# IMMachinations/Task-Vector-Replication

Measured on AMD Instinct MI355X. Metric: patched-forward prompts/sec, Pythia-2.8B layer×head CIE sweep, 1–8 GPUs, higher is better.
Workload: dtype f32 (x2f16 emulation: fp32 activations as 2 fp16 planes against the checkpoint's exact fp16 weights, 2 MFMA products, fp32 accumulate); 1 GPU; pythia-2.8b CIE sweep 32x32 sites, 12 prompts/step, 4-shot, T=15, fp16-valued weights (exact-fp16 GEMMs, 2 products); parallelism=single GPU, gemm=x2f16, weights=fp16, exact16_gemms=True

## Files before the change

include/tvr.h:

```cpp
#ifndef TVR_H_
#define TVR_H_

#include <stddef.h>
#include <stdint.h>

#ifdef __cplusplus
extern "C" {
#endif

#define TVR_ABI_VERSION 11

enum tvr_status {
  TVR_OK = 0,
  TVR_ERR_INVALID = -1,
  TVR_ERR_HIP = -2,
  TVR_ERR_NOMEM = -3,
  TVR_ERR_UNSUPPORTED = -4,
  TVR_ERR_RANGE = -5,
  TVR_ERR_INTERNAL = -6
};

enum tvr_site_kind {
  TVR_SITE_NONE = 0,
  TVR_SITE_REPLACE_HEAD_ALLPOS = 1,
  TVR_SITE_ADD_ATTN_OUT_LASTPOS = 2,
  TVR_SITE_SET_RESID_PRE_POS = 3,
  TVR_SITE_REPLACE_HEADSET_ALLPOS = 4,
  TVR_SITE_REPLACE_HEADSET_LASTPOS = 5,
  TVR_SITE_SET_RESID_PRE_VEC = 6
};

typedef struct tvr_config {
  int32_t n_layers;
  int32_t d_model;
  int32_t n_heads;
  int32_t d_head;
  int32_t d_mlp;
  int32_t d_vocab;
  int32_t rotary_dim;
  int32_t n_ctx;
  float ln_eps;
  float rotary_base;
} tvr_config;

typedef struct tvr_layer_weights {
  const float* w1;
  const float* b1;
  const float* w2;
  const float* b2;
} tvr_layer_weights;

typedef struct tvr_site {
  int32_t seq;
  int32_t kind;
  int32_t layer;
  int32_t head;
  int32_t pos;
  int32_t src_seq;
  int32_t src_pos;
  int32_t vec;
  int32_t target;
} tvr_site;

typedef struct tvr_model tvr_model;
typedef struct tvr_trace tvr_trace;

const char* tvr_version(void);
int32_t tvr_abi_version(void);
const char* tvr_last_error(void);

int tvr_model_create(const tvr_config* cfg, const float* w_embed ,
                     const tvr_layer_weights* layers ,
                     const float* w_unembed_t ,
                     const float* b_unembed , tvr_model** out);
int tvr_model_destroy(tvr_model* model);

enum tvr_gemm_mode { TVR_GEMM_F32 = 0, TVR_GEMM_X3BF16 = 1, TVR_GEMM_X2F16 = 2, TVR_GEMM_BF16 = 3 };
int tvr_model_set_gemm(tvr_model* model, int32_t mode, void* stream);
int32_t tvr_model_get_gemm(const tvr_model* model);
int tvr_model_range_status(tvr_model* model, void* stream);

typedef struct {
  const uint16_t* w1;
  const uint16_t* w2;
  const float* g1;
  const float* g2;
} tvr_exact16_layer;
int tvr_model_set_exact16(tvr_model* model, const tvr_exact16_layer* layers );
int tvr_model_set_exact16_unembed(tvr_model* model, const uint16_t* wu, const float* gf);

int tvr_trace_create(tvr_model* model, int32_t max_seqs, int32_t max_tokens,
                     tvr_trace** out);
int tvr_trace_destroy(tvr_trace* trace);
int tvr_trace_flush(tvr_trace* trace, void* stream);
enum tvr_trace_hook { TVR_TRACE_RESID_PRE = 0, TVR_TRACE_Z = 1, TVR_TRACE_Q = 2, TVR_TRACE_K = 3, TVR_TRACE_V = 4 };
int tvr_trace_read(const tvr_trace* trace, int32_t what, int32_t layer, float* dst,
                   void* stream);
int32_t tvr_trace_num_tokens(const tvr_trace* trace);
int tvr_trace_capture_resid(tvr_trace* trace, const int32_t* pos, const int32_t* group,
                            int32_t n_groups, float* out, void* stream);
int tvr_trace_capture_pattern(tvr_trace* trace, const int32_t* pos, const int32_t* cls, int32_t n_classes,
                              float* out_pattern, int32_t ld, float* out_mass, void* stream);

int tvr_trace_logit_attribution(tvr_trace* trace, const int32_t* pos, const int32_t* target,
                                const int32_t* contrast, float* out_head, float* out_resid, void* stream);
int tvr_trace_logit_lens(tvr_trace* trace, const int32_t* pos, const int32_t* targets, float* out_prob,
                         int32_t* out_topk, int32_t topk, void* stream);

int tvr_forward_clean(tvr_model* model, tvr_trace* trace, const int32_t* tokens,
                      const int32_t* seq_lens, int32_t n_seq,
                      const int32_t* targets, float* out_prob,
                      int32_t* out_topk, int32_t topk, float* out_logits,
                      float* capture_zsum, void* stream);

int tvr_forward_clean_deferred(tvr_model* model, tvr_trace* trace, const int32_t* tokens,
                               const int32_t* seq_lens, int32_t n_seq,
                               const int32_t* targets, float* out_prob,
                               int32_t* out_topk, int32_t topk, void* stream);

int tvr_forward_logits(tvr_model* model, const int32_t* tokens, const float* resid_in,
                       int32_t start_layer, const int32_t* seq_lens, int32_t n_seq,
                       float* out_logits, void* stream);

int tvr_patch_sweep(tvr_model* model, tvr_trace* trace,
                    const tvr_site* sites, int32_t n_sites,
                    const float* vectors, int32_t n_vectors, float* out_prob,
                    int32_t* out_topk, int32_t topk, float* out_logits,
                    void* stream);

typedef struct tvr_head_patch { int32_t layer, head, vec; } tvr_head_patch;
int tvr_patch_sweep_sets(tvr_model* model, tvr_trace* trace,
                         const tvr_site* sites, int32_t n_sites,
                         const int32_t* set_off, const tvr_head_patch* patches,
                         const float* vectors, int32_t n_vectors, float* out_prob,
                         int32_t* out_topk, int32_t topk, float* out_logits,
                         void* stream);

int tvr_project_heads(tvr_model* model, const float* zsum ,
                      float* out , void* stream);

int tvr_gemm_f32(const float* A, int32_t lda, const float* W, int32_t ldw,
                 const float* bias, float* C, int32_t ldc, int32_t M,
                 int32_t N, int32_t K, void* stream);
int tvr_split_planes(const float* w, uint16_t* out, size_t n, void* stream);
int tvr_gemm_x3bf16(const float* A, int32_t lda, const uint16_t* W, int32_t ldw,
                    size_t wps, const float* bias, float* C, int32_t ldc,
                    int32_t M, int32_t N, int32_t K, void* stream);
int tvr_weight_planes(int32_t fmt, const float* w, float scale, uint16_t* out, size_t n,
                      void* stream);
int tvr_gemm_x2f16(const float* A, int32_t lda, const uint16_t* W, int32_t ldw,
                   size_t wps, float w_scale, const float* bias, float* C,
                   int32_t ldc, int32_t M, int32_t N, int32_t K,
                   uint32_t* range_flag, void* stream);
#define TVR_ACT_X2F16_IL 0x12
int tvr_act_rows(int32_t fmt, const float* a, int32_t lda, uint16_t* out, int32_t rows,
                 int32_t K, uint32_t* range_flag, void* stream);
int tvr_gemm_planar(int32_t fmt, const uint16_t* A, int32_t lda, const uint16_t* W,
                    int32_t ldw, size_t wps, float w_scale, const float* bias,
                    float* C, int32_t ldc, int32_t M, int32_t N, int32_t K,
                    void* stream);
int tvr_lnpre_f32(const float* x, int32_t ldx, float* y, int32_t ldy,
                  int32_t rows, int32_t d, float eps, void* stream);
typedef struct tvr_attn_seq { int32_t row0, n, p0, cache_row, q0, prefix_live; } tvr_attn_seq;
int tvr_attention(tvr_model* model, int32_t fmt, const float* qkv, const float* cache,
                  const tvr_attn_seq* seqs, int32_t n_seq, int32_t row_from, int32_t rows,
                  int32_t cache_rows, void* z, float* zf, int32_t zf_last, int32_t zf_rows,
                  const float* cos_t, const float* sin_t, void* stream);
int tvr_attention_pattern(tvr_model* model, const float* qkv, int32_t rows, const int32_t* row0,
                          const int32_t* qpos, int32_t n_seq, const int32_t* cls, int32_t n_classes,
                          float* out_pattern, int32_t ld, float* out_mass, const float* cos_t,
                          const float* sin_t, void* stream);
int tvr_head_attribution(tvr_model* model, int32_t layer, const float* z, const float* dirs, int32_t n,
                         float* out, void* stream);
int tvr_decode_rows(tvr_model* model, const float* rows, int32_t n, const int32_t* targets, float* out_prob,
                    int32_t* out_topk, int32_t topk, void* stream);
enum tvr_gemm_epi { TVR_EPI_BIAS = 0, TVR_EPI_GELU = 1, TVR_EPI_RESID = 2 };
enum tvr_gemm_form { TVR_FORM_PLAN = 0, TVR_FORM_PLAIN = 1, TVR_FORM_SPLITK = 2, TVR_FORM_TAIL = 3,
                     TVR_FORM_STREAMK = 4 };
enum tvr_gemm_slicing { TVR_SLICE_MODEL = 0, TVR_SLICE_ON = 1, TVR_SLICE_OFF = 2 };
typedef struct tvr_gemm_args {
  int32_t fmt, exact16, epi, form, form_n, form_tile, slicing, skinny;
  int32_t M, N, K, lda, ldw, ld0, n_split, ld1h;
  int32_t ps1h, raw_rows, ld_raw, mirror_rows, ldr, a2_col, a_buf_rows, out_buf_rows;
  float w_scale;
  int32_t reserved;
  uint64_t wps;
  const uint16_t* A;
  const uint16_t* a2;
  const uint16_t* W;
  const float* bias;
  float* out0;
  float* out0m;
  uint16_t* out1h;
  float* raw;
  const float* resid;
  uint32_t* range_flag;
  const int32_t* a_rows;
  const int32_t* out_rows;
} tvr_gemm_args;
int tvr_gemm_launch(tvr_model* model, const tvr_gemm_args* args, void* stream);

enum { TVR_ENTRY_FORCE_VALU = 1 };
int tvr_site_entry(tvr_model* model, const int32_t* seq_lens, int32_t n_seq, const int32_t* token_ids,
                   int32_t tokens, const float* resid, const float* z, const tvr_site* sites,
                   int32_t n_sites, const int32_t* set_off, const tvr_head_patch* patches,
                   const float* vectors, int32_t n_vectors, int32_t flags, float* out, int32_t out_rows,
                   int32_t* site_row0, int32_t* site_rows, int32_t* site_p0, void* stream);

typedef struct tvr_headset_item { int32_t row0, n_rows, first_patch, n_patches; } tvr_headset_item;
typedef struct tvr_headset_patch { int32_t head, vec; } tvr_headset_patch;
int tvr_headset_apply(tvr_model* model, int32_t fmt, const tvr_headset_item* items, int32_t n_items,
                      const tvr_headset_patch* patches, int32_t n_patches, const float* vectors,
                      int32_t n_vectors, void* a2, float* resid, int32_t rows, void* stream);

typedef struct tvr_kernel_stats {
  int64_t gemm_launches[3];
  double gemm_flops[3];
  double gemm_ms[3];
  double gemm_bytes[3];
} tvr_kernel_stats;
int tvr_profile_enable(tvr_model* model, int32_t on);
int tvr_profile_read(tvr_model* model, tvr_kernel_stats* out);

enum tvr_hbm_kind {
  TVR_HBM_ENTRY = 0,
  TVR_HBM_CAPTURE = 1,
  TVR_HBM_LNPRE = 2,
  TVR_HBM_ATTENTION = 3,
  TVR_HBM_ROW_STATS = 4,
  TVR_HBM_LIN_ENTRY = 5,
  TVR_HBM_KINDS = 6
};
typedef struct tvr_hbm_stats {
  int64_t launches[6];
  double ms[6];
  double bytes[6];
} tvr_hbm_stats;
int tvr_profile_read_hbm(tvr_model* model, tvr_hbm_stats* out);

// ... 11 lines not shown
```

task-vector-replication_amd/_lib.py:

```python
from __future__ import annotations

import ctypes
import os
from pathlib import Path

LIB_NAME = "libtvr.so"
OPS_NAME = "_tvr_ops.so"
LIB_PATH = Path(os.environ["TVR_LIB"]).resolve() if os.environ.get("TVR_LIB") else Path(__file__).resolve().parent / LIB_NAME

TVR_OK = 0
TVR_ERR_INVALID = -1
TVR_ERR_HIP = -2
TVR_ERR_NOMEM = -3
TVR_ERR_UNSUPPORTED = -4
TVR_ERR_RANGE = -5
TVR_ERR_INTERNAL = -6

TRACE_RESID_PRE = 0
TRACE_Z = 1
TRACE_Q = 2
TRACE_K = 3
TRACE_V = 4

SITE_NONE = 0
SITE_REPLACE_HEAD_ALLPOS = 1
SITE_ADD_ATTN_OUT_LASTPOS = 2
SITE_SET_RESID_PRE_POS = 3
SITE_REPLACE_HEADSET_ALLPOS = 4
SITE_REPLACE_HEADSET_LASTPOS = 5
SITE_SET_RESID_PRE_VEC = 6

c_f32p = ctypes.c_void_p
c_i32p = ctypes.c_void_p


class CLayerWeights(ctypes.Structure):
    _fields_ = [("w1", ctypes.c_void_p), ("b1", ctypes.c_void_p),
                ("w2", ctypes.c_void_p), ("b2", ctypes.c_void_p)]


class CExact16Layer(ctypes.Structure):
    _fields_ = [("w1", ctypes.c_void_p), ("w2", ctypes.c_void_p), ("g1", ctypes.c_void_p), ("g2", ctypes.c_void_p)]


class CSite(ctypes.Structure):
    _fields_ = [("seq", ctypes.c_int32), ("kind", ctypes.c_int32), ("layer", ctypes.c_int32),
                ("head", ctypes.c_int32), ("pos", ctypes.c_int32), ("src_seq", ctypes.c_int32),
                ("src_pos", ctypes.c_int32), ("vec", ctypes.c_int32), ("target", ctypes.c_int32)]


SITE_FIELDS = [f for f, _ in CSite._fields_]


class CHeadPatch(ctypes.Structure):
    _fields_ = [("layer", ctypes.c_int32), ("head", ctypes.c_int32), ("vec", ctypes.c_int32)]


class CHeadsetItem(ctypes.Structure):
    _fields_ = [("row0", ctypes.c_int32), ("n_rows", ctypes.c_int32), ("first_patch", ctypes.c_int32),
                ("n_patches", ctypes.c_int32)]


class CHeadsetPatch(ctypes.Structure):
    _fields_ = [("head", ctypes.c_int32), ("vec", ctypes.c_int32)]


ENTRY_FORCE_VALU = 1


class CAttnSeq(ctypes.Structure):
    _fields_ = [("row0", ctypes.c_int32), ("n", ctypes.c_int32), ("p0", ctypes.c_int32),
                ("cache_row", ctypes.c_int32), ("q0", ctypes.c_int32), ("prefix_live", ctypes.c_int32)]


ACT_X2F16_IL = 0x12


class CGemmArgs(ctypes.Structure):
    _fields_ = ([(n, ctypes.c_int32) for n in (
        "fmt", "exact16", "epi", "form", "form_n", "form_tile", "slicing", "skinny",
        "M", "N", "K", "lda", "ldw", "ld0", "n_split", "ld1h",
        "ps1h", "raw_rows", "ld_raw", "mirror_rows", "ldr", "a2_col", "a_buf_rows", "out_buf_rows")] +
                [("w_scale", ctypes.c_float), ("reserved", ctypes.c_int32), ("wps", ctypes.c_uint64)] +
                [(n, ctypes.c_void_p) for n in (
                    "A", "a2", "W", "bias", "out0", "out0m", "out1h", "raw", "resid", "range_flag",
                    "a_rows", "out_rows")])


EPI_BIAS, EPI_GELU, EPI_RESID = 0, 1, 2
FORM_PLAN, FORM_PLAIN, FORM_SPLITK, FORM_TAIL, FORM_STREAMK = 0, 1, 2, 3, 4
SLICE_MODEL, SLICE_ON, SLICE_OFF = 0, 1, 2


class CKernelStats(ctypes.Structure):
    _fields_ = [("gemm_launches", ctypes.c_int64 * 3), ("gemm_flops", ctypes.c_double * 3),
                ("gemm_ms", ctypes.c_double * 3), ("gemm_bytes", ctypes.c_double * 3)]


GEMM_VARIANTS = ("unembed", "qkv_mlpin", "o_mlpout")


class CHbmStats(ctypes.Structure):
    _fields_ = [("launches", ctypes.c_int64 * 6), ("ms", ctypes.c_double * 6), ("bytes", ctypes.c_double * 6)]


HBM_KINDS = ("entry", "capture", "lnpre", "attention", "row_stats", "lin_entry")

ABI_VERSION = 11

GEMM_MODES = {"f32": 0, "x3bf16": 1, "x2f16": 2, "bf16": 3}
GEMM_NAMES = {v: k for k, v in GEMM_MODES.items()}

SIGNATURES = {
    "tvr_version": (ctypes.c_char_p, []),
    "tvr_abi_version": (ctypes.c_int32, []),
    "tvr_last_error": (ctypes.c_char_p, []),
    "tvr_model_create": (ctypes.c_int, [ctypes.c_void_p, c_f32p, ctypes.POINTER(CLayerWeights),
                                        c_f32p, c_f32p, ctypes.POINTER(ctypes.c_void_p)]),
    "tvr_model_destroy": (ctypes.c_int, [ctypes.c_void_p]),
    "tvr_trace_create": (ctypes.c_int, [ctypes.c_void_p, ctypes.c_int32, ctypes.c_int32,
                                        ctypes.POINTER(ctypes.c_void_p)]),
    "tvr_trace_destroy": (ctypes.c_int, [ctypes.c_void_p]),
    "tvr_trace_flush": (ctypes.c_int, [ctypes.c_void_p, ctypes.c_void_p]),
    "tvr_trace_read": (ctypes.c_int, [ctypes.c_void_p, ctypes.c_int32, ctypes.c_int32, c_f32p,
                                      ctypes.c_void_p]),
    "tvr_trace_num_tokens": (ctypes.c_int32, [ctypes.c_void_p]),
    "tvr_trace_capture_resid": (ctypes.c_int, [ctypes.c_void_p, c_i32p, c_i32p, ctypes.c_int32, c_f32p,
                                               ctypes.c_void_p]),
    "tvr_forward_clean": (ctypes.c_int, [ctypes.c_void_p, ctypes.c_void_p, c_i32p, c_i32p, ctypes.c_int32,
                                         c_i32p, c_f32p, c_i32p, ctypes.c_int32, c_f32p, c_f32p,
                                         ctypes.c_void_p]),
    "tvr_forward_clean_deferred": (ctypes.c_int, [ctypes.c_void_p, ctypes.c_void_p, c_i32p, c_i32p, ctypes.c_int32,
                                                  c_i32p, c_f32p, c_i32p, ctypes.c_int32, ctypes.c_void_p]),
    "tvr_forward_logits": (ctypes.c_int, [ctypes.c_void_p, c_i32p, c_f32p, ctypes.c_int32, c_i32p, ctypes.c_int32,
                                          c_f32p, ctypes.c_void_p]),
    "tvr_patch_sweep": (ctypes.c_int, [ctypes.c_void_p, ctypes.c_void_p, ctypes.c_void_p, ctypes.c_int32,
                                       c_f32p, ctypes.c_int32, c_f32p, c_i32p, ctypes.c_int32, c_f32p,
                                       ctypes.c_void_p]),
    "tvr_patch_sweep_sets": (ctypes.c_int, [ctypes.c_void_p, ctypes.c_void_p, ctypes.c_void_p, ctypes.c_int32,
                                            c_i32p, ctypes.c_void_p, c_f32p, ctypes.c_int32, c_f32p, c_i32p,
                                            ctypes.c_int32, c_f32p, ctypes.c_void_p]),
    "tvr_project_heads": (ctypes.c_int, [ctypes.c_void_p, c_f32p, c_f32p, ctypes.c_void_p]),
    "tvr_gemm_f32": (ctypes.c_int, [c_f32p, ctypes.c_int32, c_f32p, ctypes.c_int32, c_f32p, c_f32p,
                                    ctypes.c_int32, ctypes.c_int32, ctypes.c_int32, ctypes.c_int32,
                                    ctypes.c_void_p]),
    "tvr_lnpre_f32": (ctypes.c_int, [c_f32p, ctypes.c_int32, c_f32p, ctypes.c_int32, ctypes.c_int32,
                                     ctypes.c_int32, ctypes.c_float, ctypes.c_void_p]),
    "tvr_workspace_bytes": (ctypes.c_size_t, [ctypes.c_void_p]),
    "tvr_model_set_gemm": (ctypes.c_int, [ctypes.c_void_p, ctypes.c_int32, ctypes.c_void_p]),
    "tvr_model_set_exact16": (ctypes.c_int, [ctypes.c_void_p, ctypes.c_void_p]),
    "tvr_model_set_exact16_unembed": (ctypes.c_int, [ctypes.c_void_p, ctypes.c_void_p, ctypes.c_void_p]),
    "tvr_model_get_gemm": (ctypes.c_int32, [ctypes.c_void_p]),
    "tvr_split_planes": (ctypes.c_int, [c_f32p, ctypes.c_void_p, ctypes.c_size_t, ctypes.c_void_p]),
    "tvr_gemm_x3bf16": (ctypes.c_int, [c_f32p, ctypes.c_int32, ctypes.c_void_p, ctypes.c_int32,
                                       ctypes.c_size_t, c_f32p, c_f32p, ctypes.c_int32, ctypes.c_int32,
                                       ctypes.c_int32, ctypes.c_int32, ctypes.c_void_p]),
    "tvr_model_range_status": (ctypes.c_int, [ctypes.c_void_p, ctypes.c_void_p]),
    "tvr_weight_planes": (ctypes.c_int, [ctypes.c_int32, c_f32p, ctypes.c_float, ctypes.c_void_p, ctypes.c_size_t,
                                         ctypes.c_void_p]),
    "tvr_gemm_x2f16": (ctypes.c_int, [c_f32p, ctypes.c_int32, ctypes.c_void_p, ctypes.c_int32,
                                      ctypes.c_size_t, ctypes.c_float, c_f32p, c_f32p, ctypes.c_int32,
                                      ctypes.c_int32, ctypes.c_int32, ctypes.c_int32, ctypes.c_void_p,
                                      ctypes.c_void_p]),
    "tvr_act_rows": (ctypes.c_int, [ctypes.c_int32, c_f32p, ctypes.c_int32, ctypes.c_void_p, ctypes.c_int32,
                                    ctypes.c_int32, ctypes.c_void_p, ctypes.c_void_p]),
    "tvr_gemm_planar": (ctypes.c_int, [ctypes.c_int32, ctypes.c_void_p, ctypes.c_int32, ctypes.c_void_p,
                                       ctypes.c_int32, ctypes.c_size_t, ctypes.c_float, c_f32p, c_f32p,
                                       ctypes.c_int32, ctypes.c_int32, ctypes.c_int32, ctypes.c_int32,
                                       ctypes.c_void_p]),
    "tvr_profile_enable": (ctypes.c_int, [ctypes.c_void_p, ctypes.c_int32]),
    "tvr_profile_read": (ctypes.c_int, [ctypes.c_void_p, ctypes.POINTER(CKernelStats)]),
    "tvr_profile_read_hbm": (ctypes.c_int, [ctypes.c_void_p, ctypes.POINTER(CHbmStats)]),
    "tvr_gemm_plan": (ctypes.c_int, [ctypes.c_int32, ctypes.c_int32, ctypes.c_int32, ctypes.c_int32, ctypes.c_int32,
                                     ctypes.c_void_p]),
    "tvr_attention": (ctypes.c_int, [ctypes.c_void_p, ctypes.c_int32, c_f32p, c_f32p, ctypes.c_void_p, ctypes.c_int32,
                                     ctypes.c_int32, ctypes.c_int32, ctypes.c_int32, ctypes.c_void_p, c_f32p,
                                     ctypes.c_int32, ctypes.c_int32, c_f32p, c_f32p, ctypes.c_void_p]),
    "tvr_attention_pattern": (ctypes.c_int, [ctypes.c_void_p, c_f32p, ctypes.c_int32, c_i32p, c_i32p, ctypes.c_int32,
                                             c_i32p, ctypes.c_int32, c_f32p, ctypes.c_int32, c_f32p, c_f32p, c_f32p,
                                             ctypes.c_void_p]),
    "tvr_trace_capture_pattern": (ctypes.c_int, [ctypes.c_void_p, c_i32p, c_i32p, ctypes.c_int32, c_f32p,
                                                 ctypes.c_int32, c_f32p, ctypes.c_void_p]),
    "tvr_gemm_launch": (ctypes.c_int, [ctypes.c_void_p, ctypes.POINTER(CGemmArgs), ctypes.c_void_p]),
    "tvr_head_attribution": (ctypes.c_int, [ctypes.c_void_p, ctypes.c_int32, c_f32p, c_f32p, ctypes.c_int32, c_f32p,
                                            ctypes.c_void_p]),
    "tvr_trace_logit_attribution": (ctypes.c_int, [ctypes.c_void_p, c_i32p, c_i32p, c_i32p, c_f32p, c_f32p,
                                                   ctypes.c_void_p]),
    "tvr_decode_rows": (ctypes.c_int, [ctypes.c_void_p, c_f32p, ctypes.c_int32, c_i32p, c_f32p, c_i32p,
                                       ctypes.c_int32, ctypes.c_void_p]),
    "tvr_trace_logit_lens": (ctypes.c_int, [ctypes.c_void_p, c_i32p, c_i32p, c_f32p, c_i32p, ctypes.c_int32,
                                            ctypes.c_void_p]),
    "tvr_site_entry": (ctypes.c_int, [ctypes.c_void_p, c_i32p, ctypes.c_int32, c_i32p, ctypes.c_int32, c_f32p, c_f32p,
                                      ctypes.c_void_p, ctypes.c_int32, c_i32p, ctypes.c_void_p, c_f32p,
                                      ctypes.c_int32, ctypes.c_int32, c_f32p, ctypes.c_int32, c_i32p, c_i32p, c_i32p,
                                      ctypes.c_void_p]),
    "tvr_headset_apply": (ctypes.c_int, [ctypes.c_void_p, ctypes.c_int32, ctypes.c_void_p, ctypes.c_int32,
                                         ctypes.c_void_p, ctypes.c_int32, c_f32p, ctypes.c_int32, ctypes.c_void_p,
                                         c_f32p, ctypes.c_int32, ctypes.c_void_p]),
}

OPS_PATH = LIB_PATH.parent / OPS_NAME
OPS = ("forward_clean", "patch_sweep", "project_heads", "forward_logits")
SET_OPS = ("patch_sweep_sets",)
RESID_OPS = ("capture_resid",)
PATTERN_OPS = ("capture_pattern",)
PATTERN_MAX_CLASSES = 64
ATTRIBUTION_OPS = ("head_attribution", "logit_attribution", "logit_lens", "decode_rows")
STATS_MAX_K = 16

_LIB = None
_OPS_LOADED = False


class EngineError(RuntimeError):
    pass


class RangeError(EngineError):
    """TVR_ERR_RANGE: an x2f16 GEMM input left the fp16 split's range (the
    results since the last check are not fp32-accurate).  The experiment
    functions retry on a path without that limit (``Model.range_fallback``)."""


def load(path: os.PathLike | str | None = None) -> ctypes.CDLL:
    global _LIB
    if _LIB is not None and path is None:
        return _LIB
    p = Path(path) if path else LIB_PATH
    if not p.exists():
        raise EngineError(f"{p} not found: the HIP engine is not built (no CPU fallback exists); "
                          "run `make -C task-vector-replication_amd/csrc`")
    lib = ctypes.CDLL(str(p))
    for name, (res, args) in SIGNATURES.items():
        fn = getattr(lib, name)
        fn.restype = res
# ... 35 lines not shown
```

task-vector-replication_amd/csrc/engine.hip:

```cpp
#include <hip/hip_runtime.h>

#include <algorithm>
#include <climits>
#include <cmath>
#include <cstdio>
#include <cstdlib>
#include <cstring>
#include <functional>
#include <map>
#include <string>
#include <tuple>
#include <vector>

#include "tvr.h"
#include "gemm_f32.hpp"
#include "attention_mfma.hpp"
#include "attention_pattern.hpp"
#include "logit_attribution.hpp"
#include "gemm_pingpong.hpp"
#include "gemm_skinny.hpp"
#include "gemm_planar.hpp"
#include "gemm_x2f16.hpp"
#include "gemm_x3bf16.hpp"
#include "kernels.hpp"
#include "lin_entry.hpp"
#include "entry_mfma.hpp"
#include "headset_patch.hpp"
#include "sweep_plan.hpp"

using namespace tvr;

namespace {

thread_local std::string g_last_error;

int fail(int code, const std::string& msg) {
  g_last_error = msg;
  return code;
}

#define TVR_HIP(expr)                                                           \
  do {                                                                          \
    hipError_t _e = (expr);                                                     \
    if (_e != hipSuccess)                                                       \
      return fail(TVR_ERR_HIP, std::string(#expr) + ": " + hipGetErrorString(_e)); \
  } while (0)

#define TVR_TRY(expr)        \
  do {                       \
    int _rc = (expr);        \
    if (_rc != TVR_OK) return _rc; \
  } while (0)

constexpr size_t kAlign = 256;
inline size_t align_up(size_t x) { return (x + kAlign - 1) & ~(kAlign - 1); }

struct Carve {
  size_t off = 0;
  template <class T>
  size_t take(size_t count) {
    const size_t at = off;
    off = align_up(off + count * sizeof(T));
    return at;
  }
};

struct Staging {
  void* buf[2] = {nullptr, nullptr};
  size_t cap[2] = {0, 0};
  hipEvent_t done[2] = {nullptr, nullptr};
  bool pending[2] = {false, false};
  int next = 0;
};

struct MatW {
  const float* f = nullptr;
  const uint16_t* x = nullptr;
  const uint16_t* h = nullptr;
  size_t wps = 0;
  float wscale = 1.0f;
  bool x16 = false;
  MatW rows(size_t elems) const {
    return {f ? f + elems : nullptr, x ? x + elems : nullptr, h ? h + elems : nullptr, wps, wscale, x16};
  }
};

using PlanKey = std::tuple<int, int, int, int, int, int>;
struct PpPlan {
  int ksplit = 1;
  int tail_base = 0;
  int tail_split = 1;
  int sk_base = -1;
  int sk_blocks = 0;
};
struct GemmForce {
  bool plan_set = false;
  PpPlan plan;
  int slicing = 0;
};
}

struct tvr_model {
  tvr_config cfg{};
  int D1 = 0;
  int K2 = 0;
  const float* w_embed = nullptr;
  std::vector<tvr_layer_weights> layers;
  const float* w_unembed_t = nullptr;
  const float* b_unembed = nullptr;
  float* rot_cos = nullptr;
  float* rot_sin = nullptr;
  const float** d_w2s = nullptr;
  int gemm_mode = TVR_GEMM_F32;
  uint16_t* planes = nullptr;
  unsigned* range_flag = nullptr;
  std::vector<MatW> w1, w2;
  std::vector<MatW> w1qk;
  MatW wu;
  char* ws = nullptr;
  size_t ws_bytes = 0;
  float* splitk_ws = nullptr;
  size_t splitk_bytes = 0;
  Staging staging;
  bool prof = false;
  struct ProfRec { hipEvent_t a, b; int epi; double flops, bytes; };
  std::vector<ProfRec> prof_recs;
  std::vector<hipEvent_t> prof_pool;
  int lin_mode = -1;
  int lin_failed_mode = -1;
  int lin_kp = 0;
  uint16_t* lin_planes = nullptr;
  float* lin_c1 = nullptr;
  std::vector<float> lin_scale;
  std::map<PlanKey, PpPlan> plans;
  bool x16 = false;
  bool act_il = true;
  std::vector<MatW> w1x, w2x;
  std::vector<const float*> g1, g2;
  MatW wux;
  const float* gf = nullptr;
};

struct tvr_trace {
  tvr_model* model = nullptr;
  int max_seqs = 0, max_tokens = 0;
  float* resid = nullptr;
  float* z = nullptr;
  float* qkv = nullptr;
  std::vector<int> seq_off, seq_len;
  std::vector<int32_t> tokens;
  int n_seq = 0, n_tokens = 0;
  bool pending = false;
  bool uncentred = false;
  std::vector<int32_t> p_targets;
  float* p_prob = nullptr;
  int32_t* p_topk = nullptr;
  int p_k = 0;
  void* p_stream = nullptr;
};

namespace {

constexpr int kFinalChunk = 1024;

int ensure_workspace(tvr_model* m, size_t bytes, hipStream_t st) {
  if (bytes <= m->ws_bytes) return TVR_OK;
  TVR_HIP(hipStreamSynchronize(st));
  if (m->ws) TVR_HIP(hipFree(m->ws));
  m->ws = nullptr;
  m->ws_bytes = 0;
  const size_t want = align_up(bytes + bytes / 8);
  if (hipMalloc(&m->ws, want) != hipSuccess) {
    m->ws = nullptr;
    (void)hipGetLastError();
    return fail(TVR_ERR_NOMEM, "workspace allocation of " + std::to_string(want) + " bytes failed");
  }
  m->ws_bytes = want;
  return TVR_OK;
}

int ensure_splitk(tvr_model* m, size_t bytes, hipStream_t st) {
  if (bytes <= m->splitk_bytes) return TVR_OK;
  TVR_HIP(hipStreamSynchronize(st));
  if (m->splitk_ws) TVR_HIP(hipFree(m->splitk_ws));
  m->splitk_ws = nullptr;
  m->splitk_bytes = 0;
  const size_t want = align_up(bytes);
  if (hipMalloc(&m->splitk_ws, want) != hipSuccess) {
    m->splitk_ws = nullptr;
    (void)hipGetLastError();
    return fail(TVR_ERR_NOMEM, "split-K workspace allocation of " + std::to_string(want) + " bytes failed");
  }
  m->splitk_bytes = want;
  return TVR_OK;
}

int upload(tvr_model* m, hipStream_t st, void* dst, const void* src, size_t bytes) {
  if (bytes == 0) return TVR_OK;
  Staging& s = m->staging;
  const int i = s.next;
  s.next ^= 1;
  if (s.pending[i]) {
    TVR_HIP(hipEventSynchronize(s.done[i]));
    s.pending[i] = false;
  }
  if (s.cap[i] < bytes) {
    if (s.buf[i]) TVR_HIP(hipHostFree(s.buf[i]));
    s.buf[i] = nullptr;
    const size_t want = align_up(std::max(bytes, (size_t)1 << 20));
    TVR_HIP(hipHostMalloc(&s.buf[i], want, hipHostMallocDefault));
    s.cap[i] = want;
  }
  if (!s.done[i]) TVR_HIP(hipEventCreateWithFlags(&s.done[i], hipEventDisableTiming));
  std::memcpy(s.buf[i], src, bytes);
  TVR_HIP(hipMemcpyAsync(dst, s.buf[i], bytes, hipMemcpyHostToDevice, st));
  TVR_HIP(hipEventRecord(s.done[i], st));
  s.pending[i] = true;
  return TVR_OK;
}

struct UploadBatch {
  std::vector<char> host;
  struct Item { size_t host_off; size_t dev_off; size_t bytes; };
  std::vector<Item> items;
  template <class T>
  void add(size_t dev_off, const std::vector<T>& v) {
    items.push_back({host.size(), dev_off, v.size() * sizeof(T)});
    const char* p = reinterpret_cast<const char*>(v.data());
    host.insert(host.end(), p, p + v.size() * sizeof(T));
  }
};

int flush_uploads(tvr_model* m, hipStream_t st, char* base, const UploadBatch& ub) {
  if (ub.items.empty()) return TVR_OK;
  const size_t first = ub.items.front().dev_off;
  std::vector<char> span;
  size_t end = first;
  for (const auto& it : ub.items) end = std::max(end, it.dev_off + it.bytes);
  span.assign(end - first, 0);
  for (const auto& it : ub.items)
    std::memcpy(span.data() + (it.dev_off - first), ub.host.data() + it.host_off, it.bytes);
  return upload(m, st, base + first, span.data(), span.size());
}

hipEvent_t prof_event(tvr_model* m) {
  hipEvent_t e = nullptr;
  if (!m->prof_pool.empty()) {
    e = m->prof_pool.back();
    m->prof_pool.pop_back();
  } else if (hipEventCreate(&e) != hipSuccess) {
    e = nullptr;
  }
  return e;
}

struct ProfSpan {
  tvr_model* m;
  hipStream_t st;
  hipEvent_t a = nullptr, b = nullptr;
  ProfSpan(tvr_model* m_, hipStream_t s) : m(m_), st(s) {
    if (m && m->prof) {
      a = prof_event(m);
      b = prof_event(m);
      if (a) (void)hipEventRecord(a, st);
    }
  }
  void done(int kind, double bytes) {
    if (!a || !b) return;
    (void)hipEventRecord(b, st);
    m->prof_recs.push_back({a, b, 3 + kind, 0.0, bytes});
    a = b = nullptr;
  }
  ~ProfSpan() {
    if (a) m->prof_pool.push_back(a);
    if (b) m->prof_pool.push_back(b);
  }
};

bool env_flag(const char* name) {
  const char* e = getenv(name);
  return !(e && std::string(e) == "0");
}
bool prefix_share_enabled() { return env_flag("TVR_PREFIX_SHARE"); }
bool lin_entry_enabled() { return env_flag("TVR_LIN_ENTRY"); }

int act_fmt(const tvr_model* m) {
  return m->gemm_mode == TVR_GEMM_X2F16 ? ACT_X2F16 : m->gemm_mode == TVR_GEMM_BF16 ? ACT_BF16 : ACT_F32;
}

bool use_x16(const tvr_model* m) { return m->x16 && m->gemm_mode == TVR_GEMM_X2F16; }

bool act_layout_interleaved() {
  const char* e = getenv("TVR_ACT_LAYOUT");
  return !(e && std::string(e) == "planar");
}
int acts_fmt(const tvr_model* m) { return use_x16(m) && m->act_il ? (int)ACT_X2F16I : act_fmt(m); }

int env_int(const char* name, int dflt) {
  const char* e = getenv(name);
  return e && *e ? atoi(e) : dflt;
}
int pp_group_m(int N) {
  static const int small = env_int("TVR_PP_GM_SMALL", 2), large = env_int("TVR_PP_GM_LARGE", 4);
  return (N + 255) / 256 <= 16 ? small : large;
}

void launch_pp(PpKernel kp, const uint16_t* Ah, int lda, const MatW& W, int ldw, int M, int N, int K,
               const GemmEpi& ep0, float acc_scale, int tile_base, int count, hipStream_t st) {
  GemmEpi ep = ep0;
  ep.tile_base = tile_base;
  ep.tile_count = count;
  ep.group_m = pp_group_m(N);
  const dim3 g(count > 0 ? count : gemm_pingpong_grid(M, N));
  hipLaunchKernelGGL(kp, g, dim3(PP_THREADS), 0, st, Ah, 2 * lda, (size_t)lda, W.h, ldw, W.wps, acc_scale, M, N, K, ep);
}

struct PpLaunch {
  PpKernel whole = nullptr;
  PpKernel partial = nullptr;
  PpReduceKernel reduce = nullptr;
  PpSkReduceKernel sk_reduce = nullptr;
  bool skm = false;
  int base = 0, n = 0;
};

int launch_pp_partial(const PpLaunch& pl, const uint16_t* Ah, int lda, int a_fmt, const MatW& W, int ldw, int M, int N,
                      int K, const GemmEpi& ep0, float acc_scale, int count, tvr_model* m, hipStream_t st) {
  const int n = pl.n;
  const size_t ws_tiles = pl.skm ? (size_t)2 * n : (size_t)n * count;
  const int rc = ensure_splitk(m, ws_tiles * PP_TILE_ELEMS * sizeof(float), st);
  if (rc != TVR_OK) return rc;
  GemmEpi ep = ep0;
  ep.group_m = pp_group_m(N);
  GemmEpi pe{};
  pe.group_m = ep.group_m;
  pe.out0 = m->splitk_ws;
  pe.a_rows = ep.a_rows;
  if (pl.skm) pe.sk_blocks = n; else pe.k_split = n;
  pe.tile_base = pl.base;
  pe.tile_count = count;
  pe.a2 = ep.a2;
  pe.a2_col = ep.a2_col;
  const dim3 g(pl.skm ? n : count * n);
  const dim3 rg((unsigned)std::min<long>(4096, ((long)count * (PP_TILE_ELEMS / 4) + 255) / 256));
  hipLaunchKernelGGL(pl.partial, g, dim3(PP_THREADS), 0, st, Ah, 2 * lda, (size_t)lda, W.h, ldw, W.wps, acc_scale, M,
                     N, K, pe);
  const float* part = (const float*)m->splitk_ws;
  if (pl.skm)
    hipLaunchKernelGGL(pl.sk_reduce, rg, dim3(256), 0, st, part, n, K / pp_ktile(a_fmt), pl.base, count, M, N, ep);
  else
    hipLaunchKernelGGL(pl.reduce, rg, dim3(256), 0, st, part, n, pl.base, count, M, N, ep);
  return TVR_OK;
}

int sk_mode() {
  const char* e = getenv("TVR_STREAM_K");
  return !e ? 0 : std::string(e) == "1" ? 1 : std::string(e) == "O" ? 2 : 0;
}
bool sk_enabled(int epi = EPI_BIAS) {
  const int md = sk_mode();
  return md == 1 || (md == 2 && epi == EPI_RESID);
}

struct PlanCost {
  double kt_us, pro_us, epi_us, part_us;
};

double plan_sim(int M, int N, int nkt, int t0, int cnt, int S, const PlanCost& pc) {
  const int nbm = (M + 255) / 256, nbn = (N + 255) / 256, gm = pp_group_m(N);
  const int nb = cnt * S, P = 256;
  std::vector<double> cu(P, 0.0);
  auto remap = [](int bid, int nwg) {
    const int xcd = bid & 7, q = nwg >> 3, r = nwg & 7;
    return (xcd < r ? xcd * (q + 1) : r * (q + 1) + (xcd - r) * q) + (bid >> 3);
  };
  double end = 0.0;
  for (int b = 0; b < nb; ++b) {
// ... 29 lines not shown
  PpPlan p;
  const int tiles = gemm_pingpong_grid(M, N), nkt = K / pp_ktile(a_fmt);
  const double kt_scale = wx ? (sliced ? 0.85 : 0.72) : 1.0;
  const double kt_us = (a_fmt == ACT_X2F16 ? 1.9 : 1.3) * (sliced ? 1.13 : 1.0) * kt_scale, seg_us = 15.0,
               epi_us = 10.0;
  auto sk_us = [&](int cnt) {
    const int G = (int)std::min<long long>(256, (long long)cnt * nkt);
    return std::ceil((double)cnt * nkt / G) * kt_us + 2.0 * seg_us + (cnt + 2.0 * G) * 0.0655 + 5.0;
  };
  const double round_plain_us = nkt * kt_us + epi_us;
  if (sk_enabled(epi) && (long long)tiles * nkt >= 4LL * 256) {
    const int rounds = (tiles + 255) / 256;
    const int tb = tiles - 256 * (rounds - 1);
    if (tb < 256 && sk_us(tb) + 5.0 < round_plain_us) {
      p.sk_base = tiles - tb;
      p.sk_blocks = (int)std::min<long long>(256, (long long)tb * nkt);
      return p;
    }
  }
  if (tiles <= 1024) {
    const PlanCost pc{kt_us, 3.0, epi == EPI_SPLIT_GELU_ACT ? 15.0 : 10.0, 7.0};
    double best = plan_sim(M, N, nkt, 0, tiles, 1, pc);
    for (int S = 2; S <= 16 && nkt / S >= 8 && tiles * S <= 4096; ++S) {
      const double c = plan_sim(M, N, nkt, 0, tiles, S, pc) + plan_reduce_us(M, N, 0, tiles, S);
      if (c < best * 0.97) {
        best = c;
        p.ksplit = S;
      }
    }
    if (tiles > 256) {
      const int base = 256 * ((tiles - 1) / 256), cnt = tiles - base;
      const double head = plan_sim(M, N, nkt, 0, base, 1, pc);
      for (int S = 2; S <= 16 && nkt / S >= 8; ++S) {
        const double c = head + plan_sim(M, N, nkt, base, cnt, S, pc) + plan_reduce_us(M, N, base, cnt, S);
        if (c < best * 0.97) {
          best = c;
          p.ksplit = 1;
          p.tail_base = base;
          p.tail_split = S;
        }
      }
    }
    return p;
  }
  const int rounds = (tiles + 255) / 256;
  const int tb = tiles - 256 * (rounds - 1);
  if (tb > 224) return p;
  int best = 1;
  double br = 1.0;
  for (int s = 2; s <= 16 && nkt / s >= 8; ++s) {
    const double r = std::ceil(tb * (double)s / 256.0) / s;
    if (r < br - 1e-9) {
      br = r;
      best = s;
    }
  }
  if (best < 2) return p;
  const double round_us = nkt * 2.5 * kt_scale;
  const double saved_us = (1.0 - br) * round_us;
  const double cost_us = (best + 1.0) * tb * (double)PP_TILE_ELEMS * 8.0 / 5.0e6;
  if (saved_us > 1.5 * cost_us + 10.0) {
    p.tail_base = 256 * (rounds - 1);
    p.tail_split = best;
  }
  return p;
}

PpPlan plan_pp_cached(tvr_model* m, int M, int N, int K, int a_fmt, int epi, bool wx = false) {
  const PlanKey key{M, N, K, a_fmt + (wx ? 16 : 0), epi == EPI_SPLIT_GELU_ACT ? 1 : epi == EPI_RESID ? 2 : 0, sk_mode()};
  auto it = m->plans.find(key);
  if (it != m->plans.end()) return it->second;
  const PpPlan p = plan_pp(M, N, K, a_fmt, epi, a_fmt == ACT_X2F16 && pp_sliced_rule(K, m->K2), wx);
  if (m->plans.size() > 4096) m->plans.clear();
  m->plans.emplace(key, p);
  return p;
}

int resolve_pp(const PpForm& f, const PpPlan& plan, PpLaunch& pl) {
  auto missing = [](const char* what, const PpForm& g) {
    return fail(TVR_ERR_INTERNAL, std::string("gemm: no ") + what + " is instantiated for the form epi " +
                                      std::to_string(g.epi) + ", fmt " + std::to_string(g.fmt) + ", vec " +
                                      std::to_string(g.vec) + ", stream-K " + std::to_string(g.skm) + ", sliced " +
                                      std::to_string(g.sl) + ", one weight plane " + std::to_string(g.wx) +
                                      ", interleaved A " + std::to_string(g.ail));
  };
  pl.skm = plan.sk_base >= 0;
  const bool whole_split = !pl.skm && plan.ksplit > 1, tail_split = !pl.skm && !whole_split && plan.tail_base > 0;
  pl.base = pl.skm ? plan.sk_base : tail_split ? plan.tail_base : 0;
  pl.n = pl.skm ? plan.sk_blocks : whole_split ? plan.ksplit : tail_split ? plan.tail_split : 0;
  if (pl.n == 0 || pl.base > 0) {
    PpForm whole = f;
    whole.vec = f.vec || pl.n > 0;
    pl.whole = pp_kernel(whole);
    if (!pl.whole) return missing("gemm_pingpong_kernel", whole);
  }
  if (pl.n > 0) {
    PpForm part = f;
    part.epi = EPI_BIAS;
    part.vec = true;
    part.skm = pl.skm;
    pl.partial = pp_kernel(part);
    if (!pl.partial) return missing("partial-tile gemm_pingpong_kernel", part);
    const int out_fmt = pp_reduce_fmt(f.fmt, f.ail);
    if (pl.skm)
      pl.sk_reduce = pp_reduce_kernel<true>(f.epi, out_fmt);
    else
      pl.reduce = pp_reduce_kernel<false>(f.epi, out_fmt);
    if (!pl.sk_reduce && !pl.reduce) return missing("reduce kernel", part);
  }
  return TVR_OK;
}

int launch_gemm(int epi, const void* A, int lda, int a_fmt, const MatW& W, int ldw, int M, int N,
                int K, const GemmEpi& ep, hipStream_t st, tvr_model* m = nullptr,
                unsigned* range_flag = nullptr, const GemmForce* force = nullptr) {
  if (M <= 0 || N <= 0) return TVR_OK;
  const bool ail = a_fmt == ACT_X2F16I;
  if (ail) {
    a_fmt = ACT_X2F16;
    if (!W.x16 && (epi != EPI_BIAS || m || ep.skinny))
      return fail(TVR_ERR_INVALID, "gemm: the interleaved activation layout belongs to the one-plane exact-fp16 GEMMs");
  }
  const bool planar = a_fmt != ACT_F32;
  if (planar && !W.h) return fail(TVR_ERR_INVALID, "gemm: planar activations need the planar weight planes");
  if (epi == EPI_SPLIT_GELU_ACT && !planar)
    return fail(TVR_ERR_INVALID, "gemm: the activation-format GELU epilogue belongs to the planar paths");
  if (epi == EPI_SPLIT_GELU && planar)
    return fail(TVR_ERR_INVALID, "gemm: planar paths write GELU columns in their activation format");
  if (epi == EPI_STATS && (!planar || N % 4 != 0 || !ep.stats))
    return fail(TVR_ERR_INVALID, "gemm: the fused statistics epilogue needs a planar format, N % 4 == 0 and a "
                                 "statistics buffer");
  if (a_fmt == ACT_F16 && epi != EPI_BIAS)
    return fail(TVR_ERR_INVALID, "gemm: the fp16 operand format has the plain (bias) epilogue only");
  if (W.x16 && a_fmt != ACT_X2F16)
    return fail(TVR_ERR_INVALID, "gemm: one-plane exact fp16 weights take x2f16 activations");
  if (ep.a2 && (a_fmt == ACT_F32 || ep.a2_col % 256 != 0))
    return fail(TVR_ERR_INVALID, "gemm: a second A operand needs a planar format and a 256-column boundary");
  if (K % GEMM_BK != 0 || lda % 4 != 0 || ldw % 4 != 0 || ((W.x || W.h) && ldw % 8 != 0) ||
      ((a_fmt == ACT_BF16 || a_fmt == ACT_F16) && K % 64 != 0))
    return fail(TVR_ERR_UNSUPPORTED, "gemm: K, lda, ldw must be multiples of 32/4/4 (8 for planes, K of 64 for "
                                     "bf16; K=" + std::to_string(K) + ")");
  const bool wx = a_fmt == ACT_X2F16 && W.x16;
  bool vec = false, sl = false, skinny = false;
  PpLaunch pl;
  if (planar) {
    vec = planar_epilogue_vec(epi, ep, N);
    static const int wx_slice = env_int("TVR_WX_SLICE", 1);
    sl = force && force->slicing ? a_fmt == ACT_X2F16 && force->slicing == 1
                                 : a_fmt == ACT_X2F16 && pp_sliced_rule(K, m ? m->K2 : 0) &&
                                       (!wx || wx_slice == 1 || (wx_slice == 2 && epi == EPI_RESID));
    skinny = ep.skinny && epi == EPI_BIAS && M <= SK_USE_M && !ep.out_rows && ep.k_split <= 1 && vec &&
             a_fmt != ACT_F16 && !wx && !ep.a2 && !ail;
    if (!skinny) {
      PpPlan plan;
      if (force && force->plan_set)
        plan = force->plan;
      else if (m && vec && epi != EPI_STATS)
        plan = plan_pp_cached(m, M, N, K, a_fmt, epi, wx);
      TVR_TRY(resolve_pp(PpForm{epi, a_fmt, vec || epi == EPI_STATS, false, sl, wx, ail}, plan, pl));
    }
  }
  hipEvent_t ev0 = nullptr, ev1 = nullptr;
  if (m && m->prof) {
    ev0 = prof_event(m);
    ev1 = prof_event(m);
    if (ev0) TVR_HIP(hipEventRecord(ev0, st));
  }
  const float acc_scale = a_fmt == ACT_BF16 ? 1.0f : a_fmt == ACT_F16 ? 1.0f / W.wscale : 1.0f / (W.wscale * X2_ASCALE);
  if (planar) {
    const uint16_t* Ah = static_cast<const uint16_t*>(A);
    if (skinny) {
      const dim3 g(gemm_skinny_grid(N));
#define TVR_SK(F, MT)                                                                                  \
  hipLaunchKernelGGL((gemm_skinny_kernel<F, MT>), g, dim3(SK_THREADS), 0, st, Ah, 2 * lda, (size_t)lda, W.h, \
                     ldw, W.wps, acc_scale, M, N, K, ep)
#define TVR_SK_F(F)                     \
  switch ((M + 15) / 16) {              \
    case 1: TVR_SK(F, 1); break;        \
    case 2: TVR_SK(F, 2); break;        \
    case 3: TVR_SK(F, 3); break;        \
    default: TVR_SK(F, 4); break;       \
  }
      if (a_fmt == ACT_X2F16) { TVR_SK_F(ACT_X2F16); } else { TVR_SK_F(ACT_BF16); }
#undef TVR_SK_F
#undef TVR_SK
    } else {
      if (pl.n == 0 || pl.base > 0) launch_pp(pl.whole, Ah, lda, W, ldw, M, N, K, ep, acc_scale, 0, pl.base, st);
      if (pl.n > 0)
        TVR_TRY(launch_pp_partial(pl, Ah, lda, a_fmt, W, ldw, M, N, K, ep, acc_scale,
                                  gemm_pingpong_grid(M, N) - pl.base, m, st));
    }
  } else {
    const float* Af = static_cast<const float*>(A);
    unsigned* flag = m ? m->range_flag : range_flag;
    const bool f32_sliced = !W.h && !W.x && pp_sliced_rule(K, m ? m->K2 : 0);
    const bool large = gemm_use_large(M, N) && !f32_sliced;
#define TVR_GEMM_LAUNCH(E, TL)                                                                                    \
  do {                                                                                                            \
    if (f32_sliced)                                                                                               \
      hipLaunchKernelGGL((gemm_f32_nt_kernel<E, TileSmall, F32_SLICE_KT>), dim3(gemm_grid<TileSmall>(M, N)),      \
                         dim3(TileSmall::THREADS), 0, st, Af, lda, W.f, ldw, M, N, K, ep);                        \
    else                                                                                                          \
      hipLaunchKernelGGL((gemm_f32_nt_kernel<E, TL>), dim3(gemm_grid<TL>(M, N)), dim3(TL::THREADS), 0,             \
                         st, Af, lda, W.f, ldw, M, N, K, ep);                                                     \
  } while (0)
#define TVR_X3_LAUNCH(E, TL)                                                                      \
  hipLaunchKernelGGL((gemm_x3bf16_nt_kernel<E, TL>), dim3(gemm_x3_grid<TL>(M, N)), dim3(TL::THREADS), \
                     0, st, Af, lda, W.x, ldw, W.wps, M, N, K, ep)
#define TVR_X2_LAUNCH(E, TL)                                                                         \
  hipLaunchKernelGGL((gemm_x2f16_nt_kernel<E, TL>), dim3(gemm_x2_grid<TL>(M, N)), dim3(TL::THREADS), 0, \
                     st, Af, lda, W.h, ldw, W.wps, acc_scale, flag, M, N, K, ep)
#define TVR_GEMM_PICK(E)                                                          \
  if (W.h) {                                                                      \
    if (large) TVR_X2_LAUNCH(E, X2Large); else TVR_X2_LAUNCH(E, X2Small);         \
  } else if (W.x) {                                                               \
    if (large) TVR_X3_LAUNCH(E, X3Large); else TVR_X3_LAUNCH(E, X3Small);         \
  } else {                                                                        \
    if (large) TVR_GEMM_LAUNCH(E, TileLarge); else TVR_GEMM_LAUNCH(E, TileSmall); \
  }
    switch (epi) {
      case EPI_BIAS: TVR_GEMM_PICK(EPI_BIAS); break;
      case EPI_SPLIT_GELU: TVR_GEMM_PICK(EPI_SPLIT_GELU); break;
      default: TVR_GEMM_PICK(EPI_RESID); break;
    }
#undef TVR_GEMM_PICK
#undef TVR_X2_LAUNCH
#undef TVR_X3_LAUNCH
#undef TVR_GEMM_LAUNCH
  }
  TVR_HIP(hipGetLastError());
  if (ev0 && ev1) {
    TVR_HIP(hipEventRecord(ev1, st));
    const double wbytes = W.x ? 6.0 : (a_fmt == ACT_BF16 || a_fmt == ACT_F16 ? 2.0 : 4.0);
    const double abytes = a_fmt == ACT_BF16 || a_fmt == ACT_F16 ? 2.0 : 4.0;
    const double cbytes = epi == EPI_STATS ? 4.0 * M * (double)ep.stats_tiles * (2 + 2 * ep.stats_k)
                                           : 4.0 * M * (double)N;
    const int kind = epi == EPI_SPLIT_GELU_ACT ? (int)EPI_SPLIT_GELU : epi == EPI_STATS ? (int)EPI_BIAS : epi;
    m->prof_recs.push_back({ev0, ev1, kind, 2.0 * M * N * (double)K,
                            abytes * M * (double)K + cbytes + wbytes * N * (double)K});
  }
  return TVR_OK;
}

int lin_qk_cols(const tvr_config& c) { return (2 * c.d_model) % 256 == 0 ? 2 * c.d_model : 0; }

int ensure_lin(tvr_model* m, hipStream_t st) {
  const int fmt = act_fmt(m);
  if (fmt == ACT_F32) return fail(TVR_ERR_INVALID, "lin entry: needs a planar GEMM mode");
  if (m->lin_planes && m->lin_mode == m->gemm_mode) return TVR_OK;
  if (m->lin_failed_mode == m->gemm_mode)
    return fail(TVR_ERR_NOMEM, "lin entry: the W1 W_O planes do not fit (earlier attempt)");
  const tvr_config& c = m->cfg;
  const int L = c.n_layers, d = c.d_model, H = c.n_heads, dh = c.d_head, N = m->D1;
  if (L < 3) return fail(TVR_ERR_INVALID, "lin entry: needs >= 3 layers");
  TVR_HIP(hipStreamSynchronize(st));
  if (m->lin_planes) TVR_HIP(hipFree(m->lin_planes));
  if (m->lin_c1) TVR_HIP(hipFree(m->lin_c1));
  m->lin_planes = nullptr;
  m->lin_c1 = nullptr;
  const int KP = (dh + 31) / 32 * 32, npl = fmt == ACT_X2F16 ? 2 : 1;
  const size_t per = (size_t)H * N * KP;
  float *wt = nullptr, *sc = nullptr;
  unsigned* d_max = nullptr;
  auto cleanup = [&]() {
    if (wt) (void)hipFree(wt);
    if (sc) (void)hipFree(sc);
    if (d_max) (void)hipFree(d_max);
  };
  const size_t splitk_had = m->splitk_bytes;
  for (int attempt = 0;; ++attempt) {
    bool ok = hipMalloc(&m->lin_planes, (size_t)(L - 2) * npl * per * sizeof(uint16_t)) == hipSuccess &&
              hipMalloc(&m->lin_c1, (size_t)L * N * sizeof(float)) == hipSuccess &&
              hipMalloc(&wt, (size_t)d * d * sizeof(float)) == hipSuccess &&
              hipMalloc(&sc, (size_t)N * d * sizeof(float)) == hipSuccess &&
              hipMalloc(&d_max, sizeof(unsigned)) == hipSuccess;
    if (ok && attempt > 0 && splitk_had > 0) {
      (void)hipGetLastError();
      ok = hipMalloc(&m->splitk_ws, splitk_had) == hipSuccess;
      if (ok) {
        m->splitk_bytes = splitk_had;
      } else {
        m->splitk_ws = nullptr;
      }
    }
    if (ok) break;
    (void)hipGetLastError();
    cleanup();
    wt = sc = nullptr;
    d_max = nullptr;
    if (m->lin_planes) (void)hipFree(m->lin_planes);
    if (m->lin_c1) (void)hipFree(m->lin_c1);
    m->lin_planes = nullptr;
    m->lin_c1 = nullptr;
    if (attempt == 0 && m->splitk_ws) {
      (void)hipFree(m->splitk_ws);
      m->splitk_ws = nullptr;
      m->splitk_bytes = 0;
      continue;
    }
    m->lin_failed_mode = m->gemm_mode;
    return fail(TVR_ERR_NOMEM, "lin entry: the W1 W_O planes do not fit");
  }
  m->lin_scale.assign(L, 1.0f);
  int rc = TVR_OK;
  for (int l = 1; l <= L - 2 && rc == TVR_OK; ++l) {
    hipLaunchKernelGGL(transpose_kernel, dim3((d + 31) / 32, (d + 31) / 32), dim3(32, 8), 0, st,
                       m->layers[l - 1].w2, m->K2, wt, d);
    GemmEpi e{};
    e.out0 = sc;
    e.ld0 = d;
    rc = launch_gemm(EPI_BIAS, m->layers[l].w1, d, ACT_F32, MatW{wt}, d, N, d, d, e, st);
    if (rc != TVR_OK) break;
    float scale = 1.0f;
    {
      unsigned hm = 0;
      hipError_t e2 = hipMemsetAsync(d_max, 0, sizeof(unsigned), st);
      if (e2 == hipSuccess) {
        const size_t n_abs = fmt == ACT_X2F16 ? (size_t)N * d : (size_t)2 * d * d;
        hipLaunchKernelGGL(absmax_kernel, dim3(1024), dim3(256), 0, st, sc, n_abs, d_max);
        e2 = hipGetLastError();
      }
      if (e2 == hipSuccess) e2 = hipMemcpyAsync(&hm, d_max, sizeof(unsigned), hipMemcpyDeviceToHost, st);
      if (e2 == hipSuccess) e2 = hipStreamSynchronize(st);
// ... 189 lines not shown
  const float inv_scale = 1.0f / std::sqrt((float)dh);
  const dim3 grid((unsigned)(n_seq * c.n_heads), (unsigned)n_layers), block(64);
#define TVR_PATTERN(DHV)                                                                                          \
  hipLaunchKernelGGL((attention_pattern_kernel<DHV>), grid, block, lds, st, qkv, layer_stride, 3 * d, d_seqs,      \
                     c.n_heads, d_cls, n_classes, out_pattern, ld, out_mass, rot_cos, rot_sin, d, inv_scale)
  if (dh == 16) { TVR_PATTERN(16); } else if (dh == 64) { TVR_PATTERN(64); }
  else if (dh == 80) { TVR_PATTERN(80); } else { TVR_PATTERN(128); }
#undef TVR_PATTERN
  TVR_HIP(hipGetLastError());
  return TVR_OK;
}

int check_pattern_args(const char* fn, const int32_t* cls, int n_cls, int32_t n_classes, const float* out_pattern,
                       const float* out_mass) {
  auto bad = [&](const std::string& what) { return fail(TVR_ERR_INVALID, std::string(fn) + ": " + what); };
  if (!out_pattern && !out_mass) return bad("out_pattern and out_mass are both null");
  if (out_mass && !cls) return bad("out_mass needs cls");
  if (cls) {
    if (n_classes <= 0 || n_classes > PATTERN_MAX_CLASSES)
      return bad("n_classes must be in [1, " + std::to_string(PATTERN_MAX_CLASSES) + "]");
    for (int r = 0; r < n_cls; ++r)
      if (cls[r] < -1 || cls[r] >= n_classes)
        return bad("class of row " + std::to_string(r) + " outside [-1, n_classes)");
  }
  return TVR_OK;
}

int launch_head_attribution(tvr_model* m, const char* fn, const float* dirs, int n, const float* z, size_t z_lstride,
                            const int32_t* d_zrows, int layer0, int n_layers, float* out, hipStream_t st) {
  const tvr_config& c = m->cfg;
  const int d = c.d_model, dh = c.d_head, H = c.n_heads;
  const int chunks = (n + ATTR_CHUNK - 1) / ATTR_CHUNK;
  if (!(dh == 16 || dh == 64 || dh == 80 || dh == 128) || d % 16 != 0)
    return fail(TVR_ERR_UNSUPPORTED, std::string(fn) + ": the attribution kernel covers d_head 16 / 64 / 80 / 128");
  if (H > 65535 || n_layers > 65535)
    return fail(TVR_ERR_UNSUPPORTED, std::string(fn) + ": too many heads or layers for one launch");
  ProfSpan ps(m, st);
  const dim3 grid((unsigned)chunks, (unsigned)H, (unsigned)n_layers), block(64 * ATTR_WAVES);
#define TVR_ATTR(NT)                                                                                              \
  hipLaunchKernelGGL((head_attribution_kernel<NT>), grid, block, 0, st, dirs, n, z, z_lstride, d_zrows, m->d_w2s, \
                     layer0, m->K2, out, n_layers, H, d)
  if (dh == 16) { TVR_ATTR(1); } else if (dh == 64) { TVR_ATTR(4); }
  else if (dh == 80) { TVR_ATTR(5); } else { TVR_ATTR(8); }
#undef TVR_ATTR
  TVR_HIP(hipGetLastError());
  ps.done(TVR_HBM_CAPTURE, 4.0 * n_layers * ((double)chunks * d * d + 2.0 * n * d + (double)n * H));
  return TVR_OK;
}

GemmEpi epi_qkv_mlpin(tvr_model* m, const float* b1, float* qkv, const Acts& a) {
  const bool planar = a.fmt != ACT_F32;
  const int d = m->cfg.d_model;
  GemmEpi e{};
  e.bias = b1;
  e.out0 = qkv;
  e.ld0 = 3 * d;
  e.n_split = 3 * d;
  e.out0m = a.qkv_mirror;
  e.mirror_rows = a.mirror_rows;
  if (planar) {
    e.out1h = reinterpret_cast<uint16_t*>(a.a2) + act_col_rt(a.fmt, d);
    e.ld1h = 2 * m->K2;
    e.ps1h = m->K2;
    e.range_flag = m->range_flag;
  } else {
    e.out1 = a.a2 + d;
    e.ld1 = m->K2;
  }
  return e;
}

double attention_bytes(int d, int q_rows, int kv_rows, int fmt, int zf_rows) {
  return ((double)q_rows * d + 2.0 * kv_rows * d) * 4.0 + (double)q_rows * d * (fmt == ACT_BF16 ? 2.0 : 4.0) +
         (double)zf_rows * d * 4.0;
}

int launch_w1(tvr_model* m, int l, const void* xn, int M, int c0, int N, const GemmEpi& ep, hipStream_t st,
              const void* xn2 = nullptr) {
  const int d = m->cfg.d_model;
  const int fmt = xn2 ? acts_fmt(m) : act_fmt(m);
  const int epi = fmt != ACT_F32 ? EPI_SPLIT_GELU_ACT : EPI_SPLIT_GELU;
  if (xn2) {
    if (!use_x16(m) || !act_is_x2(fmt)) return fail(TVR_ERR_INTERNAL, "launch_w1: gamma-scaled rows off the x16 path");
    const MatW W = m->w1x[l].rows((size_t)c0 * d);
    const int qkv_end = 3 * d - c0;
    if (qkv_end <= 0)
      return launch_gemm(epi, xn2, d, fmt, W, d, M, N, d, ep, st, m);
    if (qkv_end >= N)
      return launch_gemm(epi, xn, d, fmt, W, d, M, N, d, ep, st, m);
    if (qkv_end % 256 == 0) {
      GemmEpi e = ep;
      e.a2 = static_cast<const uint16_t*>(xn2);
      e.a2_col = qkv_end;
      return launch_gemm(epi, xn, d, fmt, W, d, M, N, d, e, st, m);
    }
    GemmEpi e1 = ep;
    e1.n_split = std::min(ep.n_split, qkv_end);
    TVR_TRY(launch_gemm(epi, xn, d, fmt, W, d, M, qkv_end, d, e1, st, m));
    GemmEpi e2 = ep;
    e2.bias = ep.bias ? ep.bias + qkv_end : nullptr;
    e2.out0 = ep.out0 ? ep.out0 + qkv_end : nullptr;
    if (ep.out0m) e2.out0m = ep.out0m + qkv_end;
    e2.n_split = ep.n_split - qkv_end;
    if (e2.n_split < 0) return fail(TVR_ERR_INTERNAL, "launch_w1: MLP-in columns below the GELU split");
    return launch_gemm(epi, xn2, d, fmt, W.rows((size_t)qkv_end * d), d, M, N - qkv_end, d, e2, st, m);
  }
  const int nqk = fmt == ACT_BF16 && !m->w1qk.empty() ? std::min(std::max(2 * d - c0, 0), N) : 0;
  if (nqk > 0) {
    GemmEpi e{};
    e.bias = ep.bias;
    e.out0 = ep.out0;
    e.ld0 = ep.ld0;
    e.a_rows = ep.a_rows;
    e.out_rows = ep.out_rows;
    e.out0m = ep.out0m;
    e.mirror_rows = ep.mirror_rows;
    TVR_TRY(launch_gemm(EPI_BIAS, static_cast<const uint16_t*>(xn) + d, d, ACT_F16,
                        m->w1qk[l].rows((size_t)c0 * d), d, M, nqk, d, e, st, m));
    if (nqk == N) return TVR_OK;
  }
  GemmEpi e = ep;
  if (nqk > 0) {
    e.bias = ep.bias ? ep.bias + nqk : nullptr;
    e.out0 = ep.out0 + nqk;
    if (ep.out0m) e.out0m = ep.out0m + nqk;
    e.n_split = ep.n_split - nqk;
  }
  return launch_gemm(epi, xn, d, fmt, m->w1[l].rows((size_t)(c0 + nqk) * d), d, M, N - nqk, d, e, st, m);
}

int apply_headset(tvr_model* m, const Acts& a, hipStream_t st) {
  if (a.hs_n <= 0) return TVR_OK;
  const tvr_config& c = m->cfg;
  const int d = c.d_model;
  const bool planar = a.fmt != ACT_F32;
  const size_t row_bytes = (size_t)m->K2 * 4;
  const int slice_bytes = c.d_head * (planar ? 2 : 4);
  const int n_planes = act_is_x2(a.fmt) ? 2 : 1;
  const int il = a.fmt == ACT_X2F16I;
  const size_t plane_bytes = (size_t)m->K2 * 2;
  const dim3 g(a.hs_n, (a.hs_max_rows + HEADSET_ROWS - 1) / HEADSET_ROWS);
  const bool v4 = ((uintptr_t)a.hs_vectors & 15) == 0 && d % 4 == 0;
  ProfSpan ps(m, st);
  if (v4)
    hipLaunchKernelGGL(headset_patch_kernel<true>, g, dim3(HEADSET_THREADS), 0, st, a.hs_items, a.hs_patches,
                       a.hs_vectors, (char*)a.a2, row_bytes, slice_bytes, n_planes, plane_bytes, a.resid, d, il);
  else
    hipLaunchKernelGGL(headset_patch_kernel<false>, g, dim3(HEADSET_THREADS), 0, st, a.hs_items, a.hs_patches,
                       a.hs_vectors, (char*)a.a2, row_bytes, slice_bytes, n_planes, plane_bytes, a.resid, d, il);
  TVR_HIP(hipGetLastError());
  ps.done(TVR_HBM_ENTRY, a.hs_bytes);
  return TVR_OK;
}

int run_block(tvr_model* m, int l, int R, const SeqDesc* d_seqs, int n_seqs, int maxT,
              Acts& a, float* qkv_out, const float* cache_qkv, float* zf, hipStream_t st, bool zf_last = false,
              int zf_rows = INT_MAX, int row_from = INT_MAX) {
  const tvr_config& c = m->cfg;
  const int d = c.d_model;
  const tvr_layer_weights& w = m->layers[l];
  TVR_TRY(launch_lnpre(a.resid, d, nullptr, a.xn, d, R, d, c.ln_eps, a.fmt, st, m, nullptr, a.resid_mirror,
                       a.mirror_rows, a.xn2 ? m->g1[l] : nullptr, a.xn2 ? m->g2[l] : nullptr, a.xn2));
  const GemmEpi e1 = epi_qkv_mlpin(m, w.b1, qkv_out, a);
  TVR_TRY(launch_w1(m, l, a.xn, R, 0, m->D1, e1, st, a.xn2));
  ProfSpan ps(m, st);
  TVR_TRY(launch_attention(m, qkv_out, cache_qkv, d_seqs, n_seqs, maxT, a.a2, a.fmt, zf, st, zf_last, zf_rows,
                           row_from));
  ps.done(TVR_HBM_ATTENTION, attention_bytes(d, R, R, a.fmt, zf ? (zf_last ? n_seqs : std::min(R, zf_rows)) : 0));
  return TVR_OK;
}

int run_block_last_rows(tvr_model* m, int l, int R, const SeqDesc* d_seqs, int n_seqs, int maxT, Acts& a,
                        const float* cache_qkv, const int32_t* d_last, int n_last, bool write_out,
                        float* zf, hipStream_t st, bool zf_last = false, int zf_rows = INT_MAX, int row_from = 0) {
  const tvr_config& c = m->cfg;
  const int d = c.d_model;
  const tvr_layer_weights& w = m->layers[l];
  TVR_TRY(launch_lnpre(a.resid, d, nullptr, a.xn, d, R, d, c.ln_eps, a.fmt, st, m, nullptr, a.resid_mirror,
                       a.mirror_rows, a.xn2 ? m->g1[l] : nullptr, a.xn2 ? m->g2[l] : nullptr, a.xn2));
  GemmEpi kv{};
  kv.bias = w.b1 + d;
  kv.out0 = a.qkv + d;
  kv.ld0 = 3 * d;
  kv.n_split = 2 * d;
  TVR_TRY(launch_w1(m, l, a.xn, R, d, 2 * d, kv, st, a.xn2));
  GemmEpi e1 = epi_qkv_mlpin(m, w.b1, a.qkv, a);
  e1.a_rows = d_last;
  e1.out_rows = d_last;
// ... 97 lines not shown
  return TVR_OK;
}

int check_config(const tvr_config& c) {
  if (c.n_layers <= 0 || c.d_model <= 0 || c.n_heads <= 0 || c.d_head <= 0 || c.d_mlp <= 0 ||
      c.d_vocab <= 0 || c.n_ctx <= 0)
    return fail(TVR_ERR_INVALID, "config: all sizes must be positive");
  if (c.n_heads * c.d_head != c.d_model)
    return fail(TVR_ERR_INVALID, "config: n_heads * d_head must equal d_model");
  if (c.rotary_dim < 0 || c.rotary_dim > c.d_head || (c.rotary_dim & 1))
    return fail(TVR_ERR_INVALID, "config: rotary_dim must be even and <= d_head");
  if (c.d_model % GEMM_BK != 0 || (c.d_model + c.d_mlp) % GEMM_BK != 0)
    return fail(TVR_ERR_UNSUPPORTED, "config: d_model and d_model + d_mlp must be multiples of 32");
  if (!(c.d_head == 16 || c.d_head == 64 || c.d_head == 80 || c.d_head == 128) || c.rotary_dim * 4 != c.d_head)
    return fail(TVR_ERR_UNSUPPORTED, "config: the attention kernel covers the Pythia heads: d_head 16 / 64 / 80 / "
                                     "128 with rotary_dim = d_head / 4");
  return TVR_OK;
}

}

namespace {
int flush_pending(tvr_trace* t, void* stream);
}

extern "C" {

const char* tvr_version(void) {
  return "tvr-mi355x 0.5.0 (gfx950, fp32 MFMA | fp32-accurate 3-plane bf16 / 2-plane fp16 split MFMA | bf16 MFMA)";
}
int32_t tvr_abi_version(void) { return TVR_ABI_VERSION; }
const char* tvr_last_error(void) { return g_last_error.c_str(); }

int tvr_model_create(const tvr_config* cfg, const float* w_embed, const tvr_layer_weights* layers,
                     const float* w_unembed_t, const float* b_unembed, tvr_model** out) {
  if (!cfg || !w_embed || !layers || !w_unembed_t || !out)
    return fail(TVR_ERR_INVALID, "tvr_model_create: null argument");
  TVR_TRY(check_config(*cfg));
  for (int l = 0; l < cfg->n_layers; ++l)
    if (!layers[l].w1 || !layers[l].b1 || !layers[l].w2 || !layers[l].b2)
      return fail(TVR_ERR_INVALID, "tvr_model_create: null weight in layer " + std::to_string(l));
  auto* m = new tvr_model();
  m->cfg = *cfg;
  m->D1 = 3 * cfg->d_model + cfg->d_mlp;
  m->K2 = cfg->d_model + cfg->d_mlp;
  m->w_embed = w_embed;
  m->layers.assign(layers, layers + cfg->n_layers);
  m->w_unembed_t = w_unembed_t;
  m->b_unembed = b_unembed;
  for (int l = 0; l < cfg->n_layers; ++l) {
    m->w1.push_back(MatW{layers[l].w1});
    m->w2.push_back(MatW{layers[l].w2});
  }
  m->wu = MatW{w_unembed_t};
  const int rd = std::max(cfg->rotary_dim, 2), n_ctx = cfg->n_ctx;
  std::vector<float> hc((size_t)n_ctx * rd), hs((size_t)n_ctx * rd);
  const int half = rd / 2;
  for (int p = 0; p < n_ctx; ++p)
    for (int i = 0; i < rd; ++i) {
      const float dim = (float)(i % half);
      const float freq = std::pow(cfg->rotary_base, dim / (float)half);
      const float ang = (float)p / freq;
      hc[(size_t)p * rd + i] = std::cos(ang);
      hs[(size_t)p * rd + i] = std::sin(ang);
    }
  std::vector<const float*> w2s(cfg->n_layers);
  for (int l = 0; l < cfg->n_layers; ++l) w2s[l] = layers[l].w2;
  hipError_t e = hipMalloc(&m->rot_cos, hc.size() * sizeof(float));
  if (e == hipSuccess) e = hipMalloc(&m->rot_sin, hs.size() * sizeof(float));
  if (e == hipSuccess) e = hipMalloc(&m->d_w2s, w2s.size() * sizeof(float*));
  if (e == hipSuccess) e = hipMalloc(&m->range_flag, sizeof(unsigned));
  if (e == hipSuccess) e = hipMemset(m->range_flag, 0, sizeof(unsigned));
  if (e == hipSuccess) e = hipMemcpy(m->rot_cos, hc.data(), hc.size() * sizeof(float), hipMemcpyHostToDevice);
  if (e == hipSuccess) e = hipMemcpy(m->rot_sin, hs.data(), hs.size() * sizeof(float), hipMemcpyHostToDevice);
  if (e == hipSuccess) e = hipMemcpy(m->d_w2s, w2s.data(), w2s.size() * sizeof(float*), hipMemcpyHostToDevice);
  if (e != hipSuccess) {
    tvr_model_destroy(m);
    return fail(TVR_ERR_HIP, std::string("tvr_model_create: ") + hipGetErrorString(e));
  }
  *out = m;
  return TVR_OK;
}

int tvr_model_destroy(tvr_model* m) {
  if (!m) return TVR_OK;
  (void)hipDeviceSynchronize();
  if (m->rot_cos) (void)hipFree(m->rot_cos);
  if (m->rot_sin) (void)hipFree(m->rot_sin);
  if (m->d_w2s) (void)hipFree(m->d_w2s);
  if (m->planes) (void)hipFree(m->planes);
  if (m->lin_planes) (void)hipFree(m->lin_planes);
  if (m->lin_c1) (void)hipFree(m->lin_c1);
  if (m->range_flag) (void)hipFree(m->range_flag);
  if (m->ws) (void)hipFree(m->ws);
  if (m->splitk_ws) (void)hipFree(m->splitk_ws);
  for (auto& r : m->prof_recs) {
    (void)hipEventDestroy(r.a);
    (void)hipEventDestroy(r.b);
  }
  for (auto e : m->prof_pool) (void)hipEventDestroy(e);
  for (int i = 0; i < 2; ++i) {
    if (m->staging.buf[i]) (void)hipHostFree(m->staging.buf[i]);
    if (m->staging.done[i]) (void)hipEventDestroy(m->staging.done[i]);
  }
  delete m;
  return TVR_OK;
}

size_t tvr_workspace_bytes(const tvr_model* m) { return m ? m->ws_bytes : 0; }

int32_t tvr_model_get_gemm(const tvr_model* m) { return m ? m->gemm_mode : -1; }

static int replan_x2f16(tvr_model* m) {
  if (m->gemm_mode != TVR_GEMM_X2F16) return TVR_OK;
  TVR_HIP(hipDeviceSynchronize());
  TVR_TRY(tvr_model_set_gemm(m, TVR_GEMM_F32, nullptr));
  return tvr_model_set_gemm(m, TVR_GEMM_X2F16, nullptr);
}

int tvr_model_set_exact16_unembed(tvr_model* m, const uint16_t* wu, const float* gf) {
  if (!m) return fail(TVR_ERR_INVALID, "tvr_model_set_exact16_unembed: null model");
  if (!wu != !gf) return fail(TVR_ERR_INVALID, "tvr_model_set_exact16_unembed: give both arrays or neither");
  m->wux = wu ? MatW{nullptr, nullptr, wu, 0, 1.0f, true} : MatW{};
  m->gf = gf;
  return TVR_OK;
}

int tvr_model_set_exact16(tvr_model* m, const tvr_exact16_layer* layers) {
  if (!m) return fail(TVR_ERR_INVALID, "tvr_model_set_exact16: null model");
  const tvr_config& c = m->cfg;
  if (!layers) {
    const bool was = m->x16;
    m->x16 = false;
    m->w1x.clear();
    m->w2x.clear();
    m->g1.clear();
    m->g2.clear();
    return was ? replan_x2f16(m) : TVR_OK;
  }
  for (int l = 0; l < c.n_layers; ++l)
    if (!layers[l].w1 || !layers[l].w2 || !layers[l].g1 || !layers[l].g2)
      return fail(TVR_ERR_INVALID, "tvr_model_set_exact16: null array in layer " + std::to_string(l));
  if (c.d_model % 32 != 0 || m->K2 % 32 != 0)
    return fail(TVR_ERR_UNSUPPORTED, "tvr_model_set_exact16: d_model and d_model + d_mlp must be multiples of 32");
  m->w1x.clear();
  m->w2x.clear();
  m->g1.clear();
  m->g2.clear();
  for (int l = 0; l < c.n_layers; ++l) {
    m->w1x.push_back(MatW{nullptr, nullptr, layers[l].w1, 0, 1.0f, true});
    m->w2x.push_back(MatW{nullptr, nullptr, layers[l].w2, 0, 1.0f, true});
    m->g1.push_back(layers[l].g1);
    m->g2.push_back(layers[l].g2);
  }
  m->x16 = true;
  return replan_x2f16(m);
}

int tvr_model_set_gemm(tvr_model* m, int32_t mode, void* stream) {
  if (!m) return fail(TVR_ERR_INVALID, "tvr_model_set_gemm: null model");
  if (mode != TVR_GEMM_F32 && mode != TVR_GEMM_X3BF16 && mode != TVR_GEMM_X2F16 && mode != TVR_GEMM_BF16)
    return fail(TVR_ERR_INVALID, "tvr_model_set_gemm: unknown mode " + std::to_string(mode));
  if (mode == m->gemm_mode) return TVR_OK;
  if (mode == TVR_GEMM_BF16 && (m->cfg.d_model % 64 != 0 || m->K2 % 64 != 0))
    return fail(TVR_ERR_UNSUPPORTED, "tvr_model_set_gemm: bf16 needs d_model and d_model + d_mlp multiples of 64");
  const hipStream_t st = (hipStream_t)stream;
  TVR_HIP(hipStreamSynchronize(st));
  for (auto& w : m->w1) w = MatW{w.f};
  for (auto& w : m->w2) w = MatW{w.f};
  m->w1qk.clear();
  m->wu = MatW{m->wu.f};
  if (m->planes) TVR_HIP(hipFree(m->planes));
  m->planes = nullptr;
  if (m->lin_planes) TVR_HIP(hipFree(m->lin_planes));
  if (m->lin_c1) TVR_HIP(hipFree(m->lin_c1));
  m->lin_planes = nullptr;
  m->lin_c1 = nullptr;
  m->lin_mode = -1;
  m->lin_failed_mode = -1;
  m->gemm_mode = TVR_GEMM_F32;
  if (mode == TVR_GEMM_F32) return TVR_OK;

  const tvr_config& c = m->cfg;
  const int L = c.n_layers;
  const size_t n1 = (size_t)m->D1 * c.d_model, n2 = (size_t)c.d_model * m->K2;
  const size_t nu = (size_t)c.d_vocab * c.d_model;
  const int np = mode == TVR_GEMM_X3BF16 ? 3 : mode == TVR_GEMM_X2F16 ? 2 : 1;
  const size_t nqk = (size_t)2 * c.d_model * c.d_model;
  const bool bf16_qk16 = env_int("TVR_DEBUG_BF16_QK", 1) != 0;
  const bool bf16_trunc = env_int("TVR_DEBUG_BF16_TRUNC", 0) != 0;
  const size_t total = np * ((mode == TVR_GEMM_X2F16 && m->x16 ? 0 : n1 + n2) * L + nu) +
                       (mode == TVR_GEMM_BF16 && bf16_qk16 ? nqk * L : 0);
  if (hipMalloc(&m->planes, total * sizeof(uint16_t)) != hipSuccess) {
    m->planes = nullptr;
    (void)hipGetLastError();
    return fail(TVR_ERR_NOMEM, "tvr_model_set_gemm: weight planes (" + std::to_string(total * 2) +
                                   " bytes) do not fit");
  }
  const bool skip_x16 = mode == TVR_GEMM_X2F16 && m->x16;
  std::vector<MatW*> mats;
  std::vector<size_t> sizes;
  for (int l = 0; l < L && !skip_x16; ++l) {
    mats.push_back(&m->w1[l]);
    sizes.push_back(n1);
    mats.push_back(&m->w2[l]);
    sizes.push_back(n2);
  }
  mats.push_back(&m->wu); sizes.push_back(nu);
  if (mode == TVR_GEMM_BF16 && bf16_qk16) {
    for (int l = 0; l < L; ++l) {
      mats.push_back(nullptr);
      sizes.push_back(nqk);
    }
  }
  std::vector<float> scale(mats.size(), 1.0f);
  size_t planned = 0;
  for (size_t i = 0; i < mats.size(); ++i) planned += (mats[i] ? (size_t)np : 1) * sizes[i];
  auto drop_planes = [&]() {
    (void)hipFree(m->planes);
    m->planes = nullptr;
    for (auto& w : m->w1) w = MatW{w.f};
    for (auto& w : m->w2) w = MatW{w.f};
    m->w1qk.clear();
    m->wu = MatW{m->wu.f};
  };
  if (planned != total) {
    drop_planes();
    return fail(TVR_ERR_INTERNAL, "tvr_model_set_gemm: planes planned " + std::to_string(planned) +
                                      " != allocated " + std::to_string(total));
  }
  if (mode == TVR_GEMM_X2F16 || mode == TVR_GEMM_BF16) {
    unsigned* d_max = nullptr;
    TVR_HIP(hipMalloc(&d_max, mats.size() * sizeof(unsigned)));
    std::vector<unsigned> h_max(mats.size(), 0);
    hipError_t e = hipMemsetAsync(d_max, 0, mats.size() * sizeof(unsigned), st);
    for (size_t i = 0; i < mats.size() && e == hipSuccess; ++i) {
      const float* src = mats[i] ? mats[i]->f : m->w1[i - (mats.size() - L)].f;
      if (mode == TVR_GEMM_BF16 && mats[i]) continue;
      hipLaunchKernelGGL(absmax_kernel, dim3(1024), dim3(256), 0, st, src, sizes[i], d_max + i);
      e = hipGetLastError();
    }
    if (e == hipSuccess) e = hipMemcpyAsync(h_max.data(), d_max, mats.size() * sizeof(unsigned),
                                            hipMemcpyDeviceToHost, st);
    if (e == hipSuccess) e = hipStreamSynchronize(st);
    (void)hipFree(d_max);
    if (e != hipSuccess) return fail(TVR_ERR_HIP, std::string("tvr_model_set_gemm: ") + hipGetErrorString(e));
    for (size_t i = 0; i < mats.size(); ++i) {
      float v;
      std::memcpy(&v, &h_max[i], sizeof(v));
      scale[i] = x2_weight_scale(v);
    }
  }
  uint16_t* p = m->planes;
  for (size_t i = 0; i < mats.size(); ++i) {
    const size_t n = sizes[i];
    if (!mats[i]) {
      const int l = (int)(i - (mats.size() - L));
      const float* f = m->w1[l].f;
      hipLaunchKernelGGL(f16_plane_kernel, dim3(2048), dim3(256), 0, st, f, scale[i], p, n);
      TVR_HIP(hipGetLastError());
      m->w1qk.push_back(MatW{f, nullptr, p, n, scale[i]});
      p += n;
      continue;
    }
    MatW& w = *mats[i];
    if (mode == TVR_GEMM_X3BF16) {
      hipLaunchKernelGGL(split_planes_kernel, dim3(2048), dim3(256), 0, st, w.f, p, n);
      w = MatW{w.f, p, nullptr, n, 1.0f};
    } else if (mode == TVR_GEMM_BF16) {
      hipLaunchKernelGGL(bf16_plane_kernel, dim3(2048), dim3(256), 0, st, w.f, p, n, (int)bf16_trunc);
      w = MatW{w.f, nullptr, p, n, 1.0f};
    } else {
      hipLaunchKernelGGL(split_planes_f16_kernel, dim3(2048), dim3(256), 0, st, w.f, scale[i], p, n);
      w = MatW{w.f, nullptr, p, n, scale[i]};
    }
    TVR_HIP(hipGetLastError());
    p += np * n;
  }
  if ((size_t)(p - m->planes) != total) {
    (void)hipStreamSynchronize(st);
    const size_t written = (size_t)(p - m->planes);
    drop_planes();
    return fail(TVR_ERR_INTERNAL, "tvr_model_set_gemm: planes written " + std::to_string(written) +
                                      " != allocated " + std::to_string(total));
  }
  TVR_HIP(hipMemsetAsync(m->range_flag, 0, sizeof(unsigned), st));
  TVR_HIP(hipStreamSynchronize(st));
  m->gemm_mode = mode;
  m->act_il = act_layout_interleaved();
  return TVR_OK;
}

int tvr_model_range_status(tvr_model* m, void* stream) {
  if (!m) return fail(TVR_ERR_INVALID, "tvr_model_range_status: null model");
  const hipStream_t st = (hipStream_t)stream;
  unsigned h = 0;
  TVR_HIP(hipMemcpyAsync(&h, m->range_flag, sizeof(unsigned), hipMemcpyDeviceToHost, st));
  TVR_HIP(hipStreamSynchronize(st));
  if (h == 0) return TVR_OK;
  TVR_HIP(hipMemsetAsync(m->range_flag, 0, sizeof(unsigned), st));
  TVR_HIP(hipStreamSynchronize(st));
  return fail(TVR_ERR_RANGE, "a GEMM input reached |a| >= " + std::to_string((int)(X2_FP16_OVERFLOW / X2_ASCALE)) +
                                 ", outside the fp16-split (X2F16) range; results since the last check are not "
                                 "fp32-accurate: use gemm mode x3bf16 or f32");
}

int tvr_profile_enable(tvr_model* m, int32_t on) {
  if (!m) return fail(TVR_ERR_INVALID, "tvr_profile_enable: null model");
  TVR_HIP(hipDeviceSynchronize());
  for (auto& r : m->prof_recs) {
    m->prof_pool.push_back(r.a);
    m->prof_pool.push_back(r.b);
  }
  m->prof_recs.clear();
  m->prof = on != 0;
  return TVR_OK;
}

int tvr_profile_read(tvr_model* m, tvr_kernel_stats* out) {
  if (!m || !out) return fail(TVR_ERR_INVALID, "tvr_profile_read: null argument");
  tvr_kernel_stats s{};
  for (auto& r : m->prof_recs) {
    if (r.epi >= 3) continue;
    TVR_HIP(hipEventSynchronize(r.b));
    float ms = 0.f;
    TVR_HIP(hipEventElapsedTime(&ms, r.a, r.b));
    s.gemm_launches[r.epi] += 1;
    s.gemm_flops[r.epi] += r.flops;
    s.gemm_bytes[r.epi] += r.bytes;
    s.gemm_ms[r.epi] += ms;
  }
  *out = s;
  return TVR_OK;
}

int tvr_profile_read_hbm(tvr_model* m, tvr_hbm_stats* out) {
  if (!m || !out) return fail(TVR_ERR_INVALID, "tvr_profile_read_hbm: null argument");
  tvr_hbm_stats s{};
  for (auto& r : m->prof_recs) {
    if (r.epi < 3) continue;
    TVR_HIP(hipEventSynchronize(r.b));
    float ms = 0.f;
    TVR_HIP(hipEventElapsedTime(&ms, r.a, r.b));
    const int k = r.epi - 3;
    s.launches[k] += 1;
    s.ms[k] += ms;
    s.bytes[k] += r.bytes;
  }
  *out = s;
  return TVR_OK;
}

int tvr_trace_create(tvr_model* m, int32_t max_seqs, int32_t max_tokens, tvr_trace** out) {
  if (!m || !out || max_seqs <= 0 || max_tokens <= 0)
    return fail(TVR_ERR_INVALID, "tvr_trace_create: bad argument");
  const tvr_config& c = m->cfg;
  auto* t = new tvr_trace();
  t->model = m;
  t->max_seqs = max_seqs;
  t->max_tokens = max_tokens;
  const size_t per = (size_t)max_tokens * c.d_model * sizeof(float);
  hipError_t e = hipMalloc(&t->resid, per * (c.n_layers + 1));
  if (e == hipSuccess) e = hipMalloc(&t->z, per * c.n_layers);
  if (e == hipSuccess) e = hipMalloc(&t->qkv, per * 3 * c.n_layers);
  if (e != hipSuccess) {
    (void)hipGetLastError();
    tvr_trace_destroy(t);
    return fail(TVR_ERR_NOMEM, "tvr_trace_create: device allocation failed");
  }
  *out = t;
  return TVR_OK;
}

// ... 577 lines not shown
                       bool force_valu = false) {
  tvr_model* m = cx.m;
  const SweepPlan& p = cx.p;
  const tvr_config& c = m->cfg;
  const int d = c.d_model, k0 = l > 0 ? p.cnt_le[l - 1] : 0, k1 = p.cnt_le[l];
  if (k1 <= k0) return TVR_OK;
  const float* snap = cx.fused ? cx.a.resid : resid_base + (size_t)l * tstride;
  const float* zsnap = l > 0 ? z_base + (size_t)(l - 1) * tstride : nullptr;
  const float* w2 = l > 0 ? m->layers[l - 1].w2 : nullptr;
  const dim3 eg(k1 - k0, (d + ENTRY_THREADS - 1) / ENTRY_THREADS);
  ProfSpan ps(m, cx.st);
  const bool mf = !force_valu && p.eg_cnt[l] > 0 &&
                  (c.d_head == 16 || c.d_head == 64 || c.d_head == 80 || c.d_head == 128);
  if (mf) {
    const dim3 gg(p.eg_cnt[l], (d + ENTRY_COLS - 1) / ENTRY_COLS);
#define TVR_ENTRY_MF(DH)                                                                                     \
  hipLaunchKernelGGL(entry_replace_mfma_kernel<DH>, gg, dim3(ENTRY_THREADS), 0, cx.st, cx.ents, cx.egidx,     \
                     cx.egroups + p.eg_beg[l], snap, zsnap, w2, m->K2, cx.vectors, cx.a.resid, d)
    switch (c.d_head) {
      case 16: TVR_ENTRY_MF(16); break;
      case 64: TVR_ENTRY_MF(64); break;
      case 80: TVR_ENTRY_MF(80); break;
      default: TVR_ENTRY_MF(128); break;
    }
#undef TVR_ENTRY_MF
    TVR_HIP(hipGetLastError());
  }
  if (p.ent_other[l] || !mf) {
    const size_t zbytes = mf ? 0 : (size_t)std::min(p.maxT, ENTRY_LDS_POS) * c.d_head * sizeof(float);
    if (zbytes > 64 * 1024)
      TVR_HIP(hipFuncSetAttribute((const void*)entry_kernel, hipFuncAttributeMaxDynamicSharedMemorySize,
                                  (int)zbytes));
    hipLaunchKernelGGL(entry_kernel, eg, dim3(ENTRY_THREADS), zbytes, cx.st, cx.ents + k0, snap, zsnap, w2, m->K2,
                       cx.vectors, cx.a.resid, d, c.d_head, mf ? 1 : 0);
    TVR_HIP(hipGetLastError());
  }
  ps.done(TVR_HBM_ENTRY, p.entry_bytes[l]);
  return TVR_OK;
}

static int sweep_block_lin(const SweepCtx& cx, int l, int Rl, const float* cache, float* zf) {
  tvr_model* m = cx.m;
  const SweepPlan& p = cx.p;
  Acts& a = cx.a;
  hipStream_t st = cx.st;
  const tvr_config& c = m->cfg;
  const tvr_layer_weights& w = m->layers[l];
  const int d = c.d_model, fmt = act_fmt(m), Rc = p.Rc, Rp = Rc + p.rows_le[l - 1], D1 = m->D1, nv = p.lin_nv[l];
  const int32_t* vids = cx.lin_vids + p.lin_vid_off[l];
  TVR_TRY(launch_lnpre(a.resid, d, nullptr, a.xn, d, Rl, d, c.ln_eps, a.fmt, st, m, cx.lnstats, a.resid_mirror,
                       a.mirror_rows, a.xn2 ? m->g1[l] : nullptr, a.xn2 ? m->g2[l] : nullptr, a.xn2));
  GemmEpi e1 = epi_qkv_mlpin(m, w.b1, a.qkv, a);
  e1.raw = cx.raw_h;
  e1.raw_rows = Rc;
  e1.ld_raw = c.d_mlp;
  TVR_TRY(launch_w1(m, l, a.xn, Rp, 0, D1, e1, st, a.xn2));
  ProfSpan ps(m, st);
  const bool prof = m->prof;
  m->prof = false;
  GemmEpi eg{};
  eg.out0 = cx.g;
  eg.ld0 = D1;
  eg.a_rows = vids;
  eg.skinny = 1;
  int rc = TVR_OK;
  const int nqk = fmt == ACT_BF16 && !m->w1qk.empty() ? 2 * d : 0;
  if (use_x16(m)) {
    uint16_t* vg1 = cx.vg;
    uint16_t* vg2 = vg1 + (size_t)2 * nv * d;
    hipLaunchKernelGGL(lin_gamma_rows_kernel, dim3((nv + 3) / 4), dim3(256), 0, st, cx.vectors, d, vids, m->g1[l],
                       m->g2[l], vg1, vg2, nv, m->range_flag);
    rc = hipGetLastError() == hipSuccess ? TVR_OK : fail(TVR_ERR_HIP, "lin_gamma_rows_kernel launch");
    GemmEpi ex = eg;
    ex.a_rows = nullptr;
    const int q = 3 * d;
    if (rc == TVR_OK && q % 256 == 0) {
      ex.a2 = vg2;
      ex.a2_col = q;
      rc = launch_gemm(EPI_BIAS, vg1, d, fmt, m->w1x[l], d, nv, D1, d, ex, st, m);
    } else if (rc == TVR_OK) {
      rc = launch_gemm(EPI_BIAS, vg1, d, fmt, m->w1x[l], d, nv, q, d, ex, st, m);
      GemmEpi e2 = ex;
      e2.out0 = ex.out0 + q;
      if (rc == TVR_OK)
        rc = launch_gemm(EPI_BIAS, vg2, d, fmt, m->w1x[l].rows((size_t)q * d), d, nv, D1 - q, d, e2, st, m);
    }
  } else if (nqk > 0) {
    rc = launch_gemm(EPI_BIAS, cx.vact + d, d, ACT_F16, m->w1qk[l], d, nv, nqk, d, eg, st, m);
    GemmEpi e2 = eg;
    e2.out0 = eg.out0 + nqk;
    if (rc == TVR_OK)
      rc = launch_gemm(EPI_BIAS, cx.vact, d, fmt, m->w1[l].rows((size_t)nqk * d), d, nv, D1 - nqk, d, e2, st, m);
  } else {
    rc = launch_gemm(EPI_BIAS, cx.vact, d, fmt, m->w1[l], d, nv, D1, d, eg, st, m);
  }
  m->prof = prof;
  TVR_TRY(rc);
  const int npl = fmt == ACT_X2F16 ? 2 : 1, KP = m->lin_kp, nmb = p.lin_nmb[l];
  const size_t per = (size_t)c.n_heads * D1 * KP;
  const uint16_t* wp = m->lin_planes + (size_t)(l - 1) * npl * per;
  const int n_ct = (D1 + 255) / 256, ct_qk = fmt == ACT_BF16 ? lin_qk_cols(c) / 256 : 0;
  float acc_scale = fmt == ACT_X2F16 ? 1.0f / (m->lin_scale[l] * X2_ASCALE) : 1.0f;
  dim3 g;
  int ct_base = 0;
#define TVR_LIN(F, NK, ...)                                                                                          \
  hipLaunchKernelGGL((lin_entry_kernel<F, NK __VA_OPT__(,) __VA_ARGS__>), g, dim3(LIN_THREADS), 0, st,                \
                     cx.lin_mbs + p.lin_mb_off[l], nmb, cx.lin_rows, wp, per, acc_scale,                              \
                     cx.trace->z + (size_t)(l - 1) * cx.trace->max_tokens * d, d, c.d_head, cx.lnstats, a.qkv,        \
                     cx.raw_h, c.d_mlp, cx.g, m->lin_c1 + (size_t)l * D1, w.b1, D1,                                   \
                     reinterpret_cast<uint16_t*>(a.a2) + act_col_rt(a.fmt, d), 2 * m->K2, m->K2, m->range_flag, ct_base)
#define TVR_LIN_K(F, ...)                                                 \
  if (KP == 32) TVR_LIN(F, 1 __VA_OPT__(,) __VA_ARGS__);                  \
  else if (KP == 64) TVR_LIN(F, 2 __VA_OPT__(,) __VA_ARGS__);             \
  else if (KP == 96) TVR_LIN(F, 3 __VA_OPT__(,) __VA_ARGS__);             \
  else TVR_LIN(F, 4 __VA_OPT__(,) __VA_ARGS__)
  if (fmt == ACT_X2F16 && a.fmt == ACT_X2F16I) {
    g = dim3(nmb * n_ct);
    TVR_LIN_K(ACT_X2F16, true);
  } else if (fmt == ACT_X2F16) {
    g = dim3(nmb * n_ct);
    TVR_LIN_K(ACT_X2F16);
  } else {
    if (ct_qk > 0) {
      g = dim3(nmb * ct_qk);
      acc_scale = 1.0f / m->lin_scale[l];
      TVR_LIN_K(ACT_F16);
    }
    g = dim3(nmb * (n_ct - ct_qk));
    acc_scale = 1.0f;
    ct_base = ct_qk;
    TVR_LIN_K(ACT_BF16);
  }
#undef TVR_LIN_K
#undef TVR_LIN
  TVR_HIP(hipGetLastError());
  ps.done(TVR_HBM_LIN_ENTRY, (double)p.lin_nrows[l] * (8.0 * D1 + 4.0 * c.d_head) + 2.0 * npl * per +
                                 nv * (8.0 * D1 + 4.0 * d) + 2.0 * npl * (double)D1 * d);
  ProfSpan pa(m, st);
  TVR_TRY(launch_attention(m, a.qkv, cache, cx.seqs, p.nc + p.cnt_le[l], p.maxT, a.a2, a.fmt, zf, st, false, Rc));
  pa.done(TVR_HBM_ATTENTION, attention_bytes(d, Rl, Rl, a.fmt, zf ? std::min(Rl, Rc) : 0));
  return run_block_out(m, l, Rl, a, st);
}

static int sweep_impl(const char* fn, tvr_model* m, tvr_trace* trace, const tvr_site* sites, int32_t n_sites,
                      const int32_t* set_off, const tvr_head_patch* patches, const float* vectors,
                      int32_t n_vectors, float* out_prob, int32_t* out_topk, int32_t topk, float* out_logits,
                      void* stream) {
  if (!m || !trace || !sites || n_sites <= 0)
    return fail(TVR_ERR_INVALID, std::string(fn) + ": bad argument");
  if (trace->model != m) return fail(TVR_ERR_INVALID, "trace belongs to another model");
  if (trace->n_seq <= 0) return fail(TVR_ERR_INVALID, "trace is empty: run tvr_forward_clean first");
  if (topk < 0 || topk > STATS_MAX_K) return fail(TVR_ERR_INVALID, "topk must be in [0, 16]");
  if (topk > 0 && !out_topk) return fail(TVR_ERR_INVALID, "topk > 0 needs out_topk");
  hipStream_t st = (hipStream_t)stream;
  const tvr_config& c = m->cfg;
  const int d = c.d_model, L = c.n_layers, fmt = act_fmt(m);
  const bool fused = trace->pending;
  if (fused) trace->uncentred = use_x16(m);

  const SweepPlanIn in{L, c.n_heads, d, c.d_head, trace->seq_off.data(), trace->seq_len.data(),
                       trace->tokens.data(), trace->n_seq, trace->n_tokens, fused,
                       prefix_share_enabled() && (int)trace->tokens.size() >= trace->n_tokens,
                       fused && fmt != ACT_F32 && L >= 3 && lin_entry_enabled(), ENTRY_GROUP, n_vectors,
                       vectors != nullptr, ((uintptr_t)vectors & 15) == 0, fmt == ACT_BF16 ? 2.0 : 4.0,
                       sites, n_sites, set_off, patches};
  SweepPlan p;
  std::string err;
  const int prc = plan_sweep(in, p, err);
// ... 197 lines not shown
  TVR_HIP(hipGetLastError());
  return TVR_OK;
}

int tvr_gemm_x3bf16(const float* A, int32_t lda, const uint16_t* W, int32_t ldw, size_t wps,
                    const float* bias, float* C, int32_t ldc, int32_t M, int32_t N, int32_t K, void* stream) {
  if (!A || !W || !C || M < 0 || N < 0 || K <= 0 || wps < (size_t)ldw * (N > 0 ? N - 1 : 0) + K)
    return fail(TVR_ERR_INVALID, "tvr_gemm_x3bf16: bad argument");
  GemmEpi e{};
  e.bias = bias;
  e.out0 = C;
  e.ld0 = ldc;
  return launch_gemm(EPI_BIAS, A, lda, ACT_F32, MatW{nullptr, W, nullptr, wps, 1.0f}, ldw, M, N, K, e,
                     (hipStream_t)stream);
}

int tvr_weight_planes(int32_t fmt, const float* w, float scale, uint16_t* out, size_t n, void* stream) {
  if (!w || !out || (fmt != TVR_GEMM_X2F16 && fmt != TVR_GEMM_BF16))
    return fail(TVR_ERR_INVALID, "tvr_weight_planes: bad argument");
  if (n == 0) return TVR_OK;
  if (fmt == TVR_GEMM_X2F16)
    hipLaunchKernelGGL(split_planes_f16_kernel, dim3(2048), dim3(256), 0, (hipStream_t)stream, w, scale, out, n);
  else
    hipLaunchKernelGGL(bf16_plane_kernel, dim3(2048), dim3(256), 0, (hipStream_t)stream, w, out, n, 0);
  TVR_HIP(hipGetLastError());
  return TVR_OK;
}

int tvr_gemm_x2f16(const float* A, int32_t lda, const uint16_t* W, int32_t ldw, size_t wps, float w_scale,
                   const float* bias, float* C, int32_t ldc, int32_t M, int32_t N, int32_t K,
                   uint32_t* range_flag, void* stream) {
  if (!A || !W || !C || M < 0 || N < 0 || K <= 0 || !(w_scale > 0.0f) ||
      wps < (size_t)ldw * (N > 0 ? N - 1 : 0) + K)
    return fail(TVR_ERR_INVALID, "tvr_gemm_x2f16: bad argument");
  GemmEpi e{};
  e.bias = bias;
  e.out0 = C;
  e.ld0 = ldc;
  return launch_gemm(EPI_BIAS, A, lda, ACT_F32, MatW{nullptr, nullptr, W, wps, w_scale}, ldw, M, N, K, e,
                     (hipStream_t)stream, nullptr, range_flag);
}

int tvr_act_rows(int32_t fmt, const float* a, int32_t lda, uint16_t* out, int32_t rows, int32_t K,
                 uint32_t* range_flag, void* stream) {
  if (!a || !out || rows < 0 || K <= 0 || lda < K ||
      (fmt != TVR_GEMM_X2F16 && fmt != TVR_GEMM_BF16 && fmt != TVR_ACT_X2F16_IL) ||
      (fmt == TVR_ACT_X2F16_IL && K % 32 != 0))
    return fail(TVR_ERR_INVALID, "tvr_act_rows: bad argument");
  const size_t n = (size_t)rows * K;
  if (n == 0) return TVR_OK;
  const dim3 grid((unsigned)std::min<size_t>((n + 255) / 256, 8192)), block(256);
  if (fmt == TVR_GEMM_X2F16)
    hipLaunchKernelGGL(act_rows_kernel<ACT_X2F16>, grid, block, 0, (hipStream_t)stream, a, lda, out, rows, K, range_flag);
  else if (fmt == TVR_ACT_X2F16_IL)
    hipLaunchKernelGGL(act_rows_kernel<ACT_X2F16I>, grid, block, 0, (hipStream_t)stream, a, lda, out, rows, K, range_flag);
  else
    hipLaunchKernelGGL(act_rows_kernel<ACT_BF16>, grid, block, 0, (hipStream_t)stream, a, lda, out, rows, K, range_flag);
  TVR_HIP(hipGetLastError());
  return TVR_OK;
}

int tvr_gemm_planar(int32_t fmt, const uint16_t* A, int32_t lda, const uint16_t* W, int32_t ldw, size_t wps,
                    float w_scale, const float* bias, float* C, int32_t ldc, int32_t M, int32_t N, int32_t K,
                    void* stream) {
  if (!A || !W || !C || M < 0 || N < 0 || K <= 0 || lda < K || !(w_scale > 0.0f) ||
      (fmt != TVR_GEMM_X2F16 && fmt != TVR_GEMM_BF16 && fmt != TVR_ACT_X2F16_IL) ||
      wps < (size_t)ldw * (N > 0 ? N - 1 : 0) + K)
    return fail(TVR_ERR_INVALID, "tvr_gemm_planar: bad argument");
  GemmEpi e{};
  e.bias = bias;
  e.out0 = C;
  e.ld0 = ldc;
  return launch_gemm(EPI_BIAS, A, lda,
                     fmt == TVR_GEMM_X2F16 ? ACT_X2F16 : fmt == TVR_ACT_X2F16_IL ? ACT_X2F16I : ACT_BF16,
                     MatW{nullptr, nullptr, W, wps, w_scale}, ldw, M, N, K, e, (hipStream_t)stream);
}

int tvr_gemm_launch(tvr_model* m, const tvr_gemm_args* a, void* stream) {
  auto bad = [](const std::string& what) { return fail(TVR_ERR_INVALID, "tvr_gemm_launch: " + what); };
  if (!m) return bad("null model");
  if (!a) return bad("null args");
  if (a->fmt != TVR_GEMM_X2F16 && a->fmt != TVR_ACT_X2F16_IL && a->fmt != TVR_GEMM_BF16)
    return bad("unknown fmt " + std::to_string(a->fmt));
  if (a->exact16 != 0 && a->exact16 != 1) return bad("exact16 must be 0 or 1");
  if (a->epi != TVR_EPI_BIAS && a->epi != TVR_EPI_GELU && a->epi != TVR_EPI_RESID)
    return bad("unknown epi " + std::to_string(a->epi));
  if (a->form < TVR_FORM_PLAN || a->form > TVR_FORM_STREAMK) return bad("unknown form " + std::to_string(a->form));
  if (a->slicing < TVR_SLICE_MODEL || a->slicing > TVR_SLICE_OFF)
    return bad("unknown slicing " + std::to_string(a->slicing));
  if (a->skinny != 0 && a->skinny != 1) return bad("skinny must be 0 or 1");
  const bool x2 = a->fmt != TVR_GEMM_BF16, il = a->fmt == TVR_ACT_X2F16_IL, x16 = a->exact16 != 0;
  if (x16 && !x2) return bad("one exact fp16 weight plane takes an x2f16 activation format");
  const int M = a->M, N = a->N, K = a->K, ktile = pp_ktile(x2 ? ACT_X2F16 : ACT_BF16);
  if (M <= 0 || N <= 0 || K <= 0) return bad("M, N and K must be positive");
  if (K % ktile != 0) return bad("K must be a multiple of the k-tile (" + std::to_string(ktile) + ")");
  if (!a->A || !a->W || !a->out0) return bad("null A, W or out0");
  if (!(a->w_scale > 0.0f) || !std::isfinite(a->w_scale)) return bad("w_scale must be positive and finite");
  if (a->lda < K || a->lda % (il ? 32 : 8) != 0)
    return bad("lda must be at least K and a multiple of 8 (32 in the interleaved layout)");
  if (a->ldw < K || a->ldw % 8 != 0) return bad("ldw must be at least K and a multiple of 8");
  const bool two_w = x2 && !x16;
  if (two_w && (a->wps % 8 != 0 || a->wps < (uint64_t)a->ldw * (N - 1) + K))
    return bad("wps must hold N rows of ldw and be a multiple of 8");
  if (a->ld0 < N) return bad("ld0 must be at least N");
  if (((uintptr_t)a->A | (uintptr_t)a->a2 | (uintptr_t)a->W | (uintptr_t)a->out0 | (uintptr_t)a->out0m |
       (uintptr_t)a->out1h | (uintptr_t)a->raw | (uintptr_t)a->resid) & 15)
    return bad("A, a2, W, out0, out0m, out1h, raw and resid must be 16-byte aligned");
  if (((uintptr_t)a->bias | (uintptr_t)a->range_flag) & 3) return bad("bias and range_flag must be 4-byte aligned");
  if (a->out_rows && a->out_buf_rows < M) return bad("out_buf_rows must be at least M under out_rows");
  const int orows = a->out_rows ? a->out_buf_rows : M;
  if (a->out_rows) {
    std::vector<char> seen(orows, 0);
    for (int r = 0; r < M; ++r) {
      const int32_t o = a->out_rows[r];
      if (o < 0 || o >= orows) return bad("out_rows[" + std::to_string(r) + "] outside [0, out_buf_rows)");
      if (seen[o]) return bad("out_rows names row " + std::to_string(o) + " twice");
      seen[o] = 1;
    }
  }
  if (a->a_rows) {
    if (a->a_buf_rows <= 0) return bad("a_buf_rows must be positive under a_rows");
    for (int r = 0; r < M; ++r)
      if (a->a_rows[r] < 0 || a->a_rows[r] >= a->a_buf_rows)
        return bad("a_rows[" + std::to_string(r) + "] outside [0, a_buf_rows)");
  }
  if (a->a2 && (a->a2_col < 0 || a->a2_col % 256 != 0)) return bad("a2_col must be a non-negative multiple of 256");
  int mask = N | a->ld0;
  if (a->epi == TVR_EPI_RESID) {
    if (!a->resid) return bad("the residual epilogue needs resid");
    if (a->ldr < N) return bad("ldr must be at least N");
    if (a->out0m) return bad("the residual epilogue has no mirror (out0m)");
    mask |= a->ldr;
  }
  if (a->out0m && (a->mirror_rows < 0 || a->mirror_rows > orows)) return bad("mirror_rows outside [0, output rows]");
  if (a->epi == TVR_EPI_GELU) {
    if (a->n_split < 0 || a->n_split > N) return bad("n_split outside [0, N]");
    const int ng = N - a->n_split;
    if (ng > 0 && !a->out1h) return bad("the GELU epilogue needs out1h");
    if (il ? a->ld1h < 64 * ((ng + 31) / 32)
           : (x2 ? a->ps1h < ng || a->ld1h < a->ps1h + ng : a->ld1h < ng) || a->ps1h < 0)
      return bad("ld1h / ps1h too small for the GELU columns");
    mask |= a->ld1h | a->ps1h | a->n_split;
    if ((mask & 3) == 0 && ((a->ld1h | a->ps1h | a->n_split) & 7) != 0)
      return bad("with the vector epilogue ld1h, ps1h and n_split must be multiples of 8");
    if (a->raw) {
      if (a->out_rows) return bad("raw is addressed by launch row: not with out_rows");
      if (a->raw_rows < 0 || a->raw_rows > M) return bad("raw_rows outside [0, M]");
      if (a->ld_raw < ng || ((mask & 3) == 0 && a->ld_raw % 4 != 0))
        return bad("ld_raw must hold the GELU columns (a multiple of 4 with the vector epilogue)");
    }
  }
  const bool vec = (mask & 3) == 0;
  const bool forced = a->form >= TVR_FORM_SPLITK;
  if (il && !x16 && (a->epi != TVR_EPI_BIAS || forced || a->skinny || a->a2))
    return bad("the interleaved layout with two weight planes runs the plain bias launch only");
  if (a->skinny && (forced || a->out0m || a->epi != TVR_EPI_BIAS))
    return bad("skinny is an opt-in of plain bias launches without a mirror");
  const int tiles = gemm_pingpong_grid(M, N), nkt = K / ktile;
  GemmForce force;
  force.slicing = a->slicing;
  if (a->form != TVR_FORM_PLAN) force.plan_set = true;
  if (forced) {
    if (!vec) return bad("a split or stream-K launch needs the vector epilogue (N and the strides multiples of 4)");
    if (a->form == TVR_FORM_STREAMK) {
      if (a->form_tile < 0 || a->form_tile >= tiles) return bad("form_tile outside the raster");
      const int cnt = tiles - a->form_tile;
      if (a->form_n < cnt || a->form_n > 256 || (long long)a->form_n > (long long)cnt * nkt)
        return bad("stream-K blocks outside [tiles, min(256, tiles x k-tiles)]");
      force.plan.sk_base = a->form_tile;
      force.plan.sk_blocks = a->form_n;
    } else {
      const bool tail = a->form == TVR_FORM_TAIL;
      if (tail && (a->form_tile < 1 || a->form_tile >= tiles)) return bad("form_tile outside the raster");
      const int cnt = tail ? tiles - a->form_tile : tiles, S = a->form_n;
      if (S < 2 || nkt / S < 8) return bad("split S must be at least 2 with at least 8 k-tiles per part");
      if ((long long)cnt * S > 4096) return bad("more partial tiles than the workspace cap (4096)");
      if (tail) {
        force.plan.tail_base = a->form_tile;
        force.plan.tail_split = S;
      } else {
        force.plan.ksplit = S;
      }
    }
  }
  const hipStream_t st = (hipStream_t)stream;
  GemmEpi e{};
  e.bias = a->bias;
  e.out0 = a->out0;
  e.ld0 = a->ld0;
  e.n_split = a->n_split;
  e.resid = a->resid;
  e.ldr = a->ldr;
  e.out1h = a->out1h;
  e.ld1h = a->ld1h;
  e.ps1h = a->ps1h;
  e.range_flag = a->range_flag;
  if (a->epi == TVR_EPI_GELU) {
    e.raw = a->raw;
    e.raw_rows = a->raw_rows;
    e.ld_raw = a->ld_raw;
  }
  e.out0m = a->out0m;
  e.mirror_rows = a->mirror_rows;
  e.a2 = a->a2;
  e.a2_col = a->a2_col;
  e.skinny = a->skinny;
  int32_t* d_rows = nullptr;
  int rc = TVR_OK;
  if (a->a_rows || a->out_rows) {
    if (hipMalloc(&d_rows, (size_t)2 * M * sizeof(int32_t)) != hipSuccess)
      return fail(TVR_ERR_NOMEM, "tvr_gemm_launch: row index buffer");
    hipError_t err = hipSuccess;
    if (a->a_rows) err = hipMemcpyAsync(d_rows, a->a_rows, (size_t)M * sizeof(int32_t), hipMemcpyHostToDevice, st);
    if (err == hipSuccess && a->out_rows)
      err = hipMemcpyAsync(d_rows + M, a->out_rows, (size_t)M * sizeof(int32_t), hipMemcpyHostToDevice, st);
    if (err == hipSuccess) err = hipStreamSynchronize(st);
    if (err != hipSuccess) rc = fail(TVR_ERR_HIP, std::string("tvr_gemm_launch: ") + hipGetErrorString(err));
    if (a->a_rows) e.a_rows = d_rows;
    if (a->out_rows) e.out_rows = d_rows + M;
  }
  if (rc == TVR_OK) {
    const int epi = a->epi == TVR_EPI_BIAS ? EPI_BIAS : a->epi == TVR_EPI_GELU ? EPI_SPLIT_GELU_ACT : EPI_RESID;
    const int afmt = il ? ACT_X2F16I : x2 ? ACT_X2F16 : ACT_BF16;
    MatW W{nullptr, nullptr, a->W, (size_t)a->wps, x2 ? a->w_scale : 1.0f, x16};
    rc = launch_gemm(epi, a->A, a->lda, afmt, W, a->ldw, M, N, K, e, st, il && !x16 ? nullptr : m, nullptr, &force);
    if (rc == TVR_OK) {
      const hipError_t err = hipGetLastError();
      if (err != hipSuccess) rc = fail(TVR_ERR_HIP, std::string("tvr_gemm_launch: ") + hipGetErrorString(err));
    }
  }
  const hipError_t err = hipStreamSynchronize(st);
  if (rc == TVR_OK && err != hipSuccess) rc = fail(TVR_ERR_HIP, std::string("tvr_gemm_launch: ") + hipGetErrorString(err));
  if (d_rows) (void)hipFree(d_rows);
  return rc;
}

int tvr_lnpre_f32(const float* x, int32_t ldx, float* y, int32_t ldy, int32_t rows, int32_t d, float eps,
                  void* stream) {
  if (!x || !y || rows < 0 || d <= 0) return fail(TVR_ERR_INVALID, "tvr_lnpre_f32: bad argument");
  return launch_lnpre(x, ldx, nullptr, y, ldy, rows, d, eps, ACT_F32, (hipStream_t)stream);
}

static_assert(sizeof(tvr_attn_seq) == sizeof(SeqDesc), "tvr_attn_seq is SeqDesc");

int tvr_attention(tvr_model* m, int32_t fmt, const float* qkv, const float* cache, const tvr_attn_seq* seqs,
                  int32_t n_seq, int32_t row_from, int32_t rows, int32_t cache_rows, void* z, float* zf,
                  int32_t zf_last, int32_t zf_rows, const float* cos_t, const float* sin_t, void* stream) {
  auto bad = [](const std::string& what) { return fail(TVR_ERR_INVALID, "tvr_attention: " + what); };
  if (!m) return bad("null model");
  if (!qkv) return bad("null qkv");
  if (!z) return bad("null z");
  if (!seqs) return bad("null seqs");
  if (n_seq <= 0) return bad("n_seq must be positive");
  if (fmt != 0 && fmt != TVR_GEMM_X2F16 && fmt != TVR_ACT_X2F16_IL && fmt != TVR_GEMM_BF16)
    return bad("unknown fmt " + std::to_string(fmt));
  if (fmt == TVR_ACT_X2F16_IL && m->K2 % 32 != 0) return bad("the interleaved format needs K2 % 32 == 0");
  if (rows <= 0 || cache_rows < 0) return bad("rows must be positive and cache_rows non-negative");
  if (zf_rows < 0) return bad("zf_rows is negative");
  if (row_from < 0 || row_from > n_seq) return bad("row_from outside [0, n_seq]");
  if ((cos_t == nullptr) != (sin_t == nullptr)) return bad("cos_t and sin_t must both be given or both be null");
  if (((uintptr_t)qkv | (uintptr_t)cache | (uintptr_t)z | (uintptr_t)zf) & 15)
    return bad("qkv, cache, z and zf must be 16-byte aligned");
  const int n_ctx = m->cfg.n_ctx;
  int maxT = 0;
  for (int s = 0; s < n_seq; ++s) {
    const tvr_attn_seq& q = seqs[s];
    const std::string at = " (sequence " + std::to_string(s) + ")";
    if (q.n < 1) return bad("n must be at least 1" + at);
    if (q.q0 < 0 || q.q0 >= q.n) return bad("q0 outside [0, n)" + at);
    if (q.p0 < 0) return bad("p0 is negative" + at);
    if ((int64_t)q.p0 + q.n > n_ctx) return bad("p0 + n exceeds n_ctx" + at);
    if (q.row0 < 0 || (int64_t)q.row0 + q.n > rows) return bad("rows [row0, row0 + n) outside the qkv buffer" + at);
    if (q.prefix_live != 0 && q.prefix_live != 1) return bad("prefix_live must be 0 or 1" + at);
    if (q.p0 > 0) {
      if (q.cache_row < 0) return bad("cache_row is negative with p0 > 0" + at);
      if (q.prefix_live == 0 && !cache) return bad("null cache with p0 > 0 and prefix_live 0" + at);
      if ((int64_t)q.cache_row + q.p0 > (q.prefix_live ? rows : cache_rows))
        return bad(std::string("prefix rows [cache_row, cache_row + p0) outside the ") +
                   (q.prefix_live ? "qkv" : "cache") + " buffer" + at);
    }
    if (s >= row_from && q.q0 != q.n - 1) return bad("a sequence at or after row_from needs q0 == n - 1" + at);
    maxT = std::max(maxT, q.p0 + q.n);
  }
  const int afmt = fmt == 0 ? ACT_F32 : fmt == TVR_GEMM_X2F16 ? ACT_X2F16 : fmt == TVR_ACT_X2F16_IL ? ACT_X2F16I : ACT_BF16;
  const hipStream_t st = (hipStream_t)stream;
  SeqDesc* d_seqs = nullptr;
  if (hipMalloc(&d_seqs, (size_t)n_seq * sizeof(SeqDesc)) != hipSuccess)
    return fail(TVR_ERR_NOMEM, "tvr_attention: descriptor buffer");
  hipError_t e = hipMemcpyAsync(d_seqs, seqs, (size_t)n_seq * sizeof(SeqDesc), hipMemcpyHostToDevice, st);
  if (e == hipSuccess) e = hipStreamSynchronize(st);
  int rc = e == hipSuccess ? TVR_OK : fail(TVR_ERR_HIP, std::string("tvr_attention: ") + hipGetErrorString(e));
  if (rc == TVR_OK)
    rc = launch_attention(m, qkv, cache, d_seqs, n_seq, maxT, z, afmt, zf, st, zf_last != 0, zf_rows, row_from, cos_t,
                          sin_t);
  e = hipStreamSynchronize(st);
  if (rc == TVR_OK && e != hipSuccess) rc = fail(TVR_ERR_HIP, std::string("tvr_attention: ") + hipGetErrorString(e));
  (void)hipFree(d_seqs);
  return rc;
}

int tvr_attention_pattern(tvr_model* m, const float* qkv, int32_t rows, const int32_t* row0, const int32_t* qpos,
                          int32_t n_seq, const int32_t* cls, int32_t n_classes, float* out_pattern, int32_t ld,
                          float* out_mass, const float* cos_t, const float* sin_t, void* stream) {
  const char* fn = "tvr_attention_pattern";
  auto bad = [&](const std::string& what) { return fail(TVR_ERR_INVALID, std::string(fn) + ": " + what); };
  if (!m) return bad("null model");
  if (!qkv) return bad("null qkv");
// ... 192 lines not shown
```

task-vector-replication_amd/csrc/gemm_pingpong.hpp:

```cpp
#pragma once
#include <hip/hip_runtime.h>
#include <stdint.h>

#include <type_traits>

#include "gemm_planar.hpp"

namespace tvr {

constexpr int PP_THREADS = 512;
constexpr int PP_TILE_ELEMS = 256 * 256;

inline int gemm_pingpong_grid(int M, int N) { return ((M + 255) / 256) * ((N + 255) / 256); }

__host__ __device__ inline void pp_tile_coords(int wg, int nbm, int nbn, int& m0, int& n0, int gm = GEMM_GROUP_M) {
  const int per_group = gm * nbn;
  const int grp = wg / per_group;
  const int first_m = grp * gm;
  const int gsz = nbm - first_m < gm ? nbm - first_m : gm;
  const int in_grp = wg - grp * per_group;
  m0 = (first_m + in_grp % gsz) * 256;
  n0 = (in_grp / gsz) * 256;
}

constexpr int PP_EPI_LDR = 260;
#ifndef TVR_PP_NT
#define TVR_PP_NT 1
#endif
constexpr bool PP_NT_STORES = TVR_PP_NT;
#ifndef TVR_PP_SLICE_MIN_K
#define TVR_PP_SLICE_MIN_K 16384
#endif
constexpr int PP_SLICE_MIN_K = TVR_PP_SLICE_MIN_K;
#ifndef TVR_PP_SLICE_FORM
#define TVR_PP_SLICE_FORM 2
#endif
#ifndef TVR_PP_SLICE_FORM_WX
#define TVR_PP_SLICE_FORM_WX 2
#endif
#ifndef TVR_PP_WX_STAGE
#define TVR_PP_WX_STAGE 0
#endif
#ifndef TVR_PP_WX_WIDE
#define TVR_PP_WX_WIDE 2
#endif
#ifndef TVR_PP_BF16_WIDE
#define TVR_PP_BF16_WIDE 0
#endif
#ifndef TVR_PP_WX_2PHASE
#define TVR_PP_WX_2PHASE 0
#endif
#ifndef TVR_PP_PF
#define TVR_PP_PF 1
#endif
__device__ __forceinline__ f32x4 slice_add(f32x4 c, f32x4 t) { return c + t; }
constexpr int PP_EPI_LDS = 128 * PP_EPI_LDR * 2;

template <int CTRL>
__device__ __forceinline__ float dpp_f(float v) {
  return __int_as_float(__builtin_amdgcn_update_dpp(0, __float_as_int(v), CTRL, 0xF, 0xF, false));
}
template <int CTRL>
__device__ __forceinline__ int dpp_i(int v) {
  return __builtin_amdgcn_update_dpp(0, v, CTRL, 0xF, 0xF, false);
}
constexpr int DPP_QUAD_X1 = 0xB1, DPP_QUAD_X2 = 0x4E;
__device__ __forceinline__ void quad_argmax(float& bv, int& bi) {
  argmax_merge(bv, bi, dpp_f<DPP_QUAD_X1>(bv), dpp_i<DPP_QUAD_X1>(bi));
  argmax_merge(bv, bi, dpp_f<DPP_QUAD_X2>(bv), dpp_i<DPP_QUAD_X2>(bi));
}
__device__ __forceinline__ void pp_stats_rows(const GemmEpi& ep, const float* L, int grow0, int col0, int rows,
                                              int Nlim, int t, float acc_scale) {
  const int r = t >> 2, q = t & 3;
  if (r >= rows) return;
  Nlim = min(Nlim, 256);
  const int K = ep.stats_k, rec = 2 + 2 * K, tile = col0 >> 8;
  const float* Lr = L + r * PP_EPI_LDR;
  const float* bias = ep.bias ? ep.bias + col0 : nullptr;
  auto elem = [&](float a, float b) { return __fadd_rn(__fmul_rn(a, acc_scale), b); };
  auto chunk = [&](int i) {
    const int c = 16 * i + 4 * q;
    const f32x4 a = *(const f32x4*)(Lr + c);
    const f32x4 b = bias ? *(const f32x4*)(bias + c) : f32x4{0.f, 0.f, 0.f, 0.f};
    return f32x4{elem(a[0], b[0]), elem(a[1], b[1]), elem(a[2], b[2]), elem(a[3], b[3])};
  };
  const int nc = (Nlim - 4 * q + 15) >> 4;
  float mx = -INFINITY;
#pragma unroll 2
  for (int i = 0; i < nc; ++i) {
// ... 553 lines not shown
#pragma unroll
        for (int j = 0; j < 4; ++j) acc[i][j] *= acc_scale;
    }
    if (has_part) {
      GemmEpi pe = ep;
      pe.out0 = part;
      pe.ld0 = 256;
      gemm_epilogue16t<EPI, OFMT, VEC, 8, 4>(pe, acc, M - m0, N - n0, wr * 128, wc * 64, lane);
    } else {
      gemm_epilogue16t<EPI, OFMT, VEC, 8, 4>(ep, acc, M, N, m0 + wr * 128, n0 + wc * 64, lane);
    }
    if (VAR == 6 && ep.stamps && t == 0) {
      unsigned long long* o = ep.stamps + 4 * blockIdx.x;
      o[0] = st0;
      o[1] = d_loop0;
      o[2] = d_loop1;
      o[3] = __builtin_amdgcn_s_memtime();
    } else if (ep.stamps && t == 0) {
      ep.stamps[2 * blockIdx.x] = __builtin_amdgcn_s_memtime() - st0;
      ep.stamps[2 * blockIdx.x + 1] = __builtin_amdgcn_s_memrealtime() - sr0;
    }
  }
}

#ifndef TVR_WT_SGB
#define TVR_WT_SGB 1
#endif
template <int EPI, int FMT, bool VEC, int VAR, bool SL, bool TWO = false, bool AIL = false, bool WIL = false>
__device__ __forceinline__ void pp_tile_wt(const uint16_t* __restrict__ A, int lda, size_t aps,
                                           const uint16_t* __restrict__ W, int ldw, float acc_scale, int M, int N,
                                           const GemmEpi& ep, int m0, int n0, int kbeg, int nk, float* part,
                                           int has_part, unsigned long long st0, unsigned long long sr0) {
  using F = PlanarFmt<FMT>;
  using frag = typename F::frag;
  constexpr int NPL = F::NPL;
  constexpr int BK = F::BK;
  constexpr int KG = BK / 32;
  constexpr int CPR = BK / 8;
  constexpr int RPP = 64 / CPR;
  constexpr int PPP = 128 / RPP;
  constexpr int WP = PPP / 8;
  constexpr int PL = 256 * BK;
  constexpr int BUF = (NPL + 1) * PL;
  constexpr int NBUF = TWO ? 3 : 2;
  static_assert(!TWO || FMT == ACT_X2F16, "three 64 KB bf16 buffers do not fit the LDS");
  static_assert(NPL * KG == 2, "two A fragments per 16-row tile per k-tile");
  static_assert(!SL || FMT == ACT_X2F16, "the sliced accumulation is an x2f16 form");
  static_assert(!AIL || FMT == ACT_X2F16, "the interleaved A layout is an x2f16 form");
  constexpr int ACPR = AIL ? 8 : CPR;
  constexpr int ARPP = 64 / ACPR;
  constexpr int ABK = ACPR * 8;
  constexpr int VM = 4 + 2 * WP, VM0 = 4 + 3 * WP;
  constexpr int DUMMY = NBUF * BUF;
  constexpr int LDS_HALVES = (NBUF * BUF + 512) > PP_EPI_LDS ? (NBUF * BUF + 512) : PP_EPI_LDS;
  static_assert(LDS_HALVES * 2 <= 160 * 1024, "LDS budget");
  __shared__ __attribute__((aligned(16))) uint16_t lds[LDS_HALVES];
  constexpr int OFMT = AIL ? (int)ACT_X2F16I : FMT;

  int t = threadIdx.x;
  asm volatile("" : "+v"(t));
  const int wave = t >> 6, lane = t & 63;
  const int wr = wave >> 1, wc = wave & 1;
  const int wave_s = __builtin_amdgcn_readfirstlane(wave);
  const uint16_t* Ab = ep.a2 != nullptr && n0 >= ep.a2_col ? ep.a2 : A;

  const uint16_t* src[4][2];
  int dst[4][2];
#pragma unroll
  for (int R = 0; R < 4; ++R) {
#pragma unroll
    for (int s = 0; s < 2; ++s) {
      const int pi = R >= 2 ? WP * wave_s + (WP > 1 ? s : 0) : 2 * wave_s + s;
      const bool ail = AIL && R < 2;
      const int plane = ail ? 0 : pi / PPP;
      const int x0 = ail ? pi * ARPP : (pi % PPP) * RPP;
      const int trow0 = R < 2 ? ((x0 >> 5) << 6) + (x0 & 31) + 32 * R : ((x0 >> 6) << 7) + (x0 & 63) + 64 * (R - 2);
      const int row = trow0 + (ail ? lane / ACPR : lane / CPR);
      const int chunk = ail ? (lane % ACPR) ^ planar_g<ACPR>(row) : (lane % CPR) ^ planar_g<CPR>(row);
      if (R < 2) {
        const int am = min(m0 + row, M - 1);
        src[R][s] = Ab + plane * aps + (size_t)(ep.a_rows ? ep.a_rows[am] : am) * lda + chunk * 8;
        dst[R][s] = plane * PL + trow0 * (AIL ? ABK : BK);
      } else {
        const int wn = min(n0 + row, N - 1);
        if constexpr (WIL)
          src[R][s] = W + (size_t)(wn >> 1) * (2 * ldw) + (wn & 1) * 32 + chunk * 8;
        else
          src[R][s] = W + (size_t)wn * ldw + chunk * 8;
        dst[R][s] = NPL * PL + trow0 * BK;
      }
    }
  }
  auto stage = [&](int R, int kt) {
    const bool live = kt < nk;
    const int koff = live ? (kbeg + kt) * ((AIL && R < 2) || (WIL && R >= 2) ? 64 : BK) : 0;
    const int boff = (TWO ? kt % 3 : kt & 1) * BUF;
#pragma unroll
    for (int s = 0; s < (R >= 2 ? WP : 2); ++s) glds16(src[R][s] + koff, lds + (live ? boff + dst[R][s] : DUMMY));
  };

  int aoff[2], woff[KG];
#pragma unroll
  for (int f = 0; f < 2; ++f) {
    const int p = NPL == 2 ? f : 0, g = NPL == 2 ? 0 : f;
    const int ra = wr * 64 + (lane & 15), c = 4 * g + (lane >> 4);
    if constexpr (AIL)
      aoff[f] = ra * ABK + (((4 * f + (lane >> 4)) ^ planar_g<ACPR>(ra)) << 3);
    else
      aoff[f] = p * PL + ra * BK + ((c ^ planar_g<CPR>(ra)) << 3);
  }
#pragma unroll
  for (int g = 0; g < KG; ++g) {
    const int rb = wc * 128 + (lane & 15), c = 4 * g + (lane >> 4);
    woff[g] = NPL * PL + rb * BK + ((c ^ planar_g<CPR>(rb)) << 3);
  }

  f32x4 acc[4][8];
#pragma unroll
  for (int i = 0; i < 4; ++i)
#pragma unroll
    for (int j = 0; j < 8; ++j) acc[i][j] = f32x4{};
  frag fa[4][2], fw[8][KG];

  const int vi = __builtin_amdgcn_readfirstlane(min(4, max(0, (M - m0 - wr * 64 + 15) >> 4)));
  auto read_a = [&](const uint16_t* base, int i0, auto part) {
#pragma unroll
    for (int i = i0; i < i0 + 2; ++i)
      if (!decltype(part)::value || i < vi)
#pragma unroll
        for (int f = 0; f < 2; ++f) fa[i][f] = *(const frag*)(base + aoff[f] + i * 16 * ABK);
  };
  auto read_w = [&](const uint16_t* base, int j0, auto part) {
    if (decltype(part)::value && vi == 0) return;
#pragma unroll
    for (int j = j0; j < j0 + 4; ++j)
#pragma unroll
      for (int g = 0; g < KG; ++g) fw[j][g] = *(const frag*)(base + woff[g] + j * 16 * BK);
  };
  [[maybe_unused]] f32x4 tc[2] = {f32x4{0.f, 0.f, 0.f, 0.f}, f32x4{0.f, 0.f, 0.f, 0.f}};
  constexpr int NJ = TWO ? 8 : 4, NP = NJ / 2;
  auto cluster = [&](int i0, int j0, auto part, int ci, int cj) {
    if constexpr (SL && !decltype(part)::value) {
      f32x4 s[2][2];
#pragma unroll
      for (int q = 0; q < 2 * NP; ++q) {
        const int i = i0 + q / NP, j = j0 + 2 * (q % NP);
        const int pi = q == 0 ? ci : i0 + (q - 1) / NP, pj = q == 0 ? cj : j0 + 2 * ((q - 1) % NP);
#pragma unroll
        for (int u = 0; u < 4; ++u) {
          const int jj = u & 1, pz = u >> 1;
          s[q & 1][jj] = __builtin_amdgcn_mfma_f32_16x16x32_f16(fw[j + jj][0], fa[i][pz == 0 ? 1 : 0],
                                                                 pz == 0 ? f32x4{0.f, 0.f, 0.f, 0.f} : s[q & 1][jj],
                                                                 0, 0, 0);
          if (TVR_WT_SGB) __builtin_amdgcn_sched_group_barrier(0x008, 1, 0);
#pragma unroll
          for (int e = 2 * u; e < 2 * u + 2; ++e)
            acc[pi][pj + (e >> 2)][e & 3] += q == 0 ? tc[e >> 2][e & 3] : s[(q - 1) & 1][e >> 2][e & 3];
          if (TVR_WT_SGB) __builtin_amdgcn_sched_group_barrier(0x002, 2, 0);
        }
        if (NP == 4 && q == NP - 1) __builtin_amdgcn_sched_barrier(0);
      }
      tc[0] = s[(2 * NP - 1) & 1][0];
      tc[1] = s[(2 * NP - 1) & 1][1];
      return;
    }
#pragma unroll
    for (int i = i0; i < i0 + 2; ++i)
#pragma unroll
      for (int j = j0; j < j0 + NJ; ++j) {
        if (decltype(part)::value && i >= vi) continue;
        f32x4 c = acc[i][j];
        if constexpr (SL) {
          f32x4 s = __builtin_amdgcn_mfma_f32_16x16x32_f16(fw[j][0], fa[i][1], f32x4{0.f, 0.f, 0.f, 0.f}, 0, 0, 0);
          s = __builtin_amdgcn_mfma_f32_16x16x32_f16(fw[j][0], fa[i][0], s, 0, 0, 0);
          c = slice_add(c, s);
        } else if constexpr (FMT == ACT_X2F16) {
          c = __builtin_amdgcn_mfma_f32_16x16x32_f16(fw[j][0], fa[i][1], c, 0, 0, 0);
          c = __builtin_amdgcn_mfma_f32_16x16x32_f16(fw[j][0], fa[i][0], c, 0, 0, 0);
// ... 196 lines not shown
      const int nk = (int)min((long long)(nk_all - kbeg), it1 - it);
      int m0, n0;
      pp_tile_coords(ep.tile_base + lt, nbm, nbn, m0, n0, gm);
      pp_tile_any<EPI, FMT, VEC, VAR, SL, WX, SKM, AIL, WIL>(A, lda, aps, W, ldw, wps, acc_scale, M, N, ep, m0, n0, kbeg, nk,
                                  ep.out0 + ((size_t)2 * g + seg) * PP_TILE_ELEMS, 1, st0, sr0);
      it += nk;
    };
    segment(0);
    if (it < it1) segment(1);
  } else {
    const int S = ep.k_split > 1 ? ep.k_split : 1;
    const int wgs = remap(blockIdx.x, count * S);
    const int lt = wgs / S, split = wgs - lt * S;
    int m0, n0;
    pp_tile_coords(ep.tile_base + lt, nbm, nbn, m0, n0, gm);
    const int kbeg = (int)((long long)split * nk_all / S);
    const int nk = (int)((long long)(split + 1) * nk_all / S) - kbeg;
    pp_tile_any<EPI, FMT, VEC, VAR, SL, WX, SKM, AIL, WIL>(A, lda, aps, W, ldw, wps, acc_scale, M, N, ep, m0, n0, kbeg, nk,
                                ep.out0 + ((size_t)split * count + lt) * PP_TILE_ELEMS, S > 1, st0, sr0);
  }
}

template <int EPI, int FMT>
__global__ void __launch_bounds__(256)
splitk_reduce_kernel(const float* __restrict__ part, int S, int tile_base, int count, int M, int N, GemmEpi ep) {
  const int nbm = (M + 255) >> 8, nbn = (N + 255) >> 8;
  const size_t total = (size_t)count * (PP_TILE_ELEMS / 4);
  for (size_t i = blockIdx.x * (size_t)blockDim.x + threadIdx.x; i < total; i += (size_t)gridDim.x * blockDim.x) {
    const int lt = (int)(i / (PP_TILE_ELEMS / 4)), e = (int)(i % (PP_TILE_ELEMS / 4)) * 4;
    int m0, n0;
    pp_tile_coords(tile_base + lt, nbm, nbn, m0, n0, ep.group_m > 0 ? ep.group_m : GEMM_GROUP_M);
    const int m = m0 + (e >> 8), c = n0 + (e & 255);
    if (m >= M || c >= N) continue;
    const float* p = part + (size_t)lt * PP_TILE_ELEMS + e;
    f32x4 v = *(const f32x4*)p;
    for (int s = 1; s < S; ++s) v += *(const f32x4*)(p + (size_t)s * count * PP_TILE_ELEMS);
    if (ep.bias) {
#pragma unroll
      for (int r = 0; r < 4; ++r) v[r] += ep.bias[c + r];
    }
    const size_t orow = ep.out_rows ? (size_t)ep.out_rows[m] : (size_t)m;
    epi_store4<EPI, FMT>(ep, orow, c, v);
  }
}

template <int EPI, int FMT>
__global__ void __launch_bounds__(256)
splitk_sk_reduce_kernel(const float* __restrict__ part, int G, int KT, int tile_base, int count, int M, int N,
                        GemmEpi ep) {
  const int nbm = (M + 255) >> 8, nbn = (N + 255) >> 8;
  const long long I = (long long)count * KT;
  const size_t total = (size_t)count * (PP_TILE_ELEMS / 4);
  for (size_t i = blockIdx.x * (size_t)blockDim.x + threadIdx.x; i < total; i += (size_t)gridDim.x * blockDim.x) {
    const int lt = (int)(i / (PP_TILE_ELEMS / 4)), e = (int)(i % (PP_TILE_ELEMS / 4)) * 4;
    int m0, n0;
    pp_tile_coords(tile_base + lt, nbm, nbn, m0, n0, ep.group_m > 0 ? ep.group_m : GEMM_GROUP_M);
    const int m = m0 + (e >> 8), c = n0 + (e & 255);
    if (m >= M || c >= N) continue;
    const long long x0 = (long long)lt * KT, x1 = x0 + KT - 1;
    const int b0 = (int)(((x0 + 1) * G - 1) / I), b1 = (int)(((x1 + 1) * G - 1) / I);
    f32x4 v = {0.f, 0.f, 0.f, 0.f};
    for (int b = b0; b <= b1; ++b) {
      const int slot = ((long long)b * I / G) < x0 ? 1 : 0;
      v += *(const f32x4*)(part + ((size_t)2 * b + slot) * PP_TILE_ELEMS + e);
    }
    if (ep.bias) {
#pragma unroll
      for (int r = 0; r < 4; ++r) v[r] += ep.bias[c + r];
    }
    const size_t orow = ep.out_rows ? (size_t)ep.out_rows[m] : (size_t)m;
    epi_store4<EPI, FMT>(ep, orow, c, v);
  }
}


inline int pp_ktile(int fmt) { return fmt == ACT_X2F16 ? PlanarFmt<ACT_X2F16>::BK : PlanarFmt<ACT_BF16>::BK; }
static_assert(PlanarFmt<ACT_F16>::BK == PlanarFmt<ACT_BF16>::BK, "pp_ktile: fp16 and bf16 share a k-tile length");

inline bool pp_sliced_rule(int K, int K2) { return K >= PP_SLICE_MIN_K || K2 >= PP_SLICE_MIN_K; }

struct PpForm {
  int epi, fmt;
  bool vec, skm, sl, wx, ail;
};
using PpKernel = void (*)(const uint16_t*, int, size_t, const uint16_t*, int, size_t, float, int, int, int, GemmEpi);

constexpr bool pp_form_exists(int epi, int fmt, bool vec, bool skm, bool sl, bool wx, bool ail) {
  if (fmt != ACT_X2F16 && (sl || wx || ail)) return false;
  if (ail && !wx && (epi != EPI_BIAS || skm)) return false;
  if (skm) return epi == EPI_BIAS && vec;
  switch (epi) {
    case EPI_BIAS: return true;
    case EPI_SPLIT_GELU_ACT:
    case EPI_RESID: return fmt != ACT_F16;
    case EPI_STATS: return fmt != ACT_F16 && vec;
    default: return false;
  }
}

template <int EPI, int FMT, bool VEC, bool SKM, bool SL, bool WX, bool AIL>
PpKernel pp_kernel_at() {
  if constexpr (pp_form_exists(EPI, FMT, VEC, SKM, SL, WX, AIL))
    return gemm_pingpong_kernel<EPI, FMT, VEC, 0, SKM, SL, WX, AIL>;
  else
    return nullptr;
}
template <int EPI, int FMT, bool... B, class... Rest>
PpKernel pp_kernel_at(bool b, Rest... rest) {
  return b ? pp_kernel_at<EPI, FMT, B..., true>(rest...) : pp_kernel_at<EPI, FMT, B..., false>(rest...);
}
template <int EPI>
PpKernel pp_kernel_epi(const PpForm& f) {
  switch (f.fmt) {
    case ACT_X2F16: return pp_kernel_at<EPI, ACT_X2F16>(f.vec, f.skm, f.sl, f.wx, f.ail);
    case ACT_BF16: return pp_kernel_at<EPI, ACT_BF16>(f.vec, f.skm, f.sl, f.wx, f.ail);
    case ACT_F16: return pp_kernel_at<EPI, ACT_F16>(f.vec, f.skm, f.sl, f.wx, f.ail);
    default: return nullptr;
  }
}
template <int VAR = 0>
PpKernel pp_kernel(const PpForm& f) {
  static_assert(VAR == 0, "the engine's forms run VAR 0");
  switch (f.epi) {
    case EPI_BIAS: return pp_kernel_epi<EPI_BIAS>(f);
    case EPI_SPLIT_GELU_ACT: return pp_kernel_epi<EPI_SPLIT_GELU_ACT>(f);
    case EPI_RESID: return pp_kernel_epi<EPI_RESID>(f);
    case EPI_STATS: return pp_kernel_epi<EPI_STATS>(f);
    default: return nullptr;
  }
}

inline int pp_reduce_fmt(int a_fmt, bool ail) { return ail ? ACT_X2F16I : a_fmt == ACT_X2F16 ? ACT_X2F16 : ACT_BF16; }
using PpReduceKernel = void (*)(const float*, int, int, int, int, int, GemmEpi);
using PpSkReduceKernel = void (*)(const float*, int, int, int, int, int, int, GemmEpi);
template <bool SK, int EPI, int FMT>
auto pp_reduce_at() {
  if constexpr (SK)
    return PpSkReduceKernel(splitk_sk_reduce_kernel<EPI, FMT>);
  else
    return PpReduceKernel(splitk_reduce_kernel<EPI, FMT>);
}
template <bool SK, int EPI>
auto pp_reduce_epi(int out_fmt) -> decltype(pp_reduce_at<SK, EPI, ACT_BF16>()) {
  switch (out_fmt) {
    case ACT_X2F16I: return pp_reduce_at<SK, EPI, ACT_X2F16I>();
    case ACT_X2F16: return pp_reduce_at<SK, EPI, ACT_X2F16>();
    case ACT_BF16: return pp_reduce_at<SK, EPI, ACT_BF16>();
    default: return nullptr;
  }
}
template <bool SK>
auto pp_reduce_kernel(int epi, int out_fmt) -> decltype(pp_reduce_at<SK, EPI_BIAS, ACT_BF16>()) {
  switch (epi) {
    case EPI_BIAS: return pp_reduce_epi<SK, EPI_BIAS>(out_fmt);
    case EPI_SPLIT_GELU_ACT: return pp_reduce_epi<SK, EPI_SPLIT_GELU_ACT>(out_fmt);
    case EPI_RESID: return pp_reduce_epi<SK, EPI_RESID>(out_fmt);
    default: return nullptr;
  }
}

}
```

task-vector-replication_amd/model.py:

```python
from __future__ import annotations

import contextlib
import ctypes
import functools
import inspect
import random
import warnings
import weakref
from dataclasses import dataclass
from typing import Dict, List, Optional, Sequence

import numpy as np
import torch

from . import _lib
from .config import CConfig, PythiaConfig, get_config
from .tokenizer import HFTokenizer, SyntheticTokenizer, TokenizerMixin
from .weights import (EngineWeights, config_from_hf_json, load_hf_safetensors, process_to_engine,
                      synth_engine_weights)

SITE_DTYPE = np.dtype([(f, np.int32) for f in _lib.SITE_FIELDS])


def range_checked(fn):
# ... 147 lines not shown
        self._x16_c = None
        self.gemm = "f32"
        self.range_fallback = True
        self.range_fallbacks: List[tuple] = []
        if weights.raw16 is not None:
            self.set_exact16(True)
        self.set_gemm(gemm)

    @classmethod
    def from_pretrained(cls, name: str, device="cuda", seed: int = 0, checkpoint: Optional[str] = None,
                        tokenizer_path: Optional[str] = None, std: float = 0.02, ln_std: float = 0.1,
                        cfg: Optional[PythiaConfig] = None, gemm: str = DEFAULT_GEMM,
                        fp16_weights: bool = False) -> "Model":
        import os
        if cfg is None:
            try:
                cfg = get_config(name)
            except ValueError:
                if not (checkpoint and os.path.isdir(checkpoint)):
                    raise
                cfg = config_from_hf_json(checkpoint)
        dev = torch.device(device)
        if checkpoint:
            w = process_to_engine(cfg, load_hf_safetensors(checkpoint, cfg), device=dev, free_source=True)
        else:
            w = synth_engine_weights(cfg, seed=seed, device=dev, std=std, ln_std=ln_std, fp16=fp16_weights)
        tok = HFTokenizer(tokenizer_path) if tokenizer_path else None
        if dev.type == "cuda":
            torch.cuda.empty_cache()
        return cls(cfg, w, tokenizer=tok, device=dev, gemm=gemm)

    @classmethod
    def from_hf_state_dict(cls, cfg: PythiaConfig, sd, device="cuda", tokenizer=None,
                           gemm: str = DEFAULT_GEMM) -> "Model":
        return cls(cfg, process_to_engine(cfg, sd, device=torch.device(device)), tokenizer, device, gemm)

    def set_gemm(self, mode: str) -> None:
        if mode not in _lib.GEMM_MODES:
            raise ValueError(f"gemm mode must be one of {sorted(_lib.GEMM_MODES)}, got {mode!r}")
        with torch.cuda.device(self.device):
            try:
                _lib.check(self._lib.tvr_model_set_gemm(self._h, _lib.GEMM_MODES[mode], self._stream()),
                           "tvr_model_set_gemm")
            finally:
                self.gemm = _lib.GEMM_NAMES.get(self._lib.tvr_model_get_gemm(self._h), mode)

    def set_exact16(self, on: bool) -> None:
        raw = self.weights.raw16
        if on and raw is None:
            raise ValueError("set_exact16: the weights are not exact in fp16 (EngineWeights.raw16 is None)")
        if on:
            for r in raw:
                for t, dt in ((r.w1, torch.float16), (r.w2, torch.float16), (r.g1, torch.float32),
                              (r.g2, torch.float32)):
                    if t.device != self.device or t.dtype != dt or not t.is_contiguous():
                        raise ValueError("raw16 tensors must be contiguous fp16 (w1, w2) / fp32 (g1, g2) on the "
                                         "model device")
            ru = self.weights.raw16_unembed
            if ru is not None:
                wu, gf = ru
                if wu.device != self.device or wu.dtype != torch.float16 or not wu.is_contiguous() or \
                        gf.device != self.device or gf.dtype != torch.float32:
                    raise ValueError("raw16_unembed must be (fp16 [V, d], fp32 [d]) contiguous on the model device")
            arr = (_lib.CExact16Layer * self.cfg.n_layers)(
                *[_lib.CExact16Layer(r.w1.data_ptr(), r.w2.data_ptr(), r.g1.data_ptr(), r.g2.data_ptr())
                  for r in raw])
        with torch.cuda.device(self.device):
            try:
                if on:
                    self._x16_c = arr
                    _lib.check(self._lib.tvr_model_set_exact16(self._h, arr), "tvr_model_set_exact16")
                    if ru is not None:
                        _lib.check(self._lib.tvr_model_set_exact16_unembed(self._h, wu.data_ptr(), gf.data_ptr()),
                                   "tvr_model_set_exact16_unembed")
                else:
                    _lib.check(self._lib.tvr_model_set_exact16_unembed(self._h, None, None),
                               "tvr_model_set_exact16_unembed")
                    _lib.check(self._lib.tvr_model_set_exact16(self._h, None), "tvr_model_set_exact16")
                    self._x16_c = None
            finally:
                self.exact16 = bool(on)
                self.gemm = _lib.GEMM_NAMES.get(self._lib.tvr_model_get_gemm(self._h), self.gemm)

    def _fall_back(self, what: str, err: Exception) -> bool:
        if self.gemm != "x2f16":
            return False
        if self.exact16:
            self.set_exact16(False)
            path = "x2f16 (processed weights)"
        else:
            self.set_gemm("x3bf16")
            path = "x3bf16"
        self.range_fallbacks.append((what, path))
        warnings.warn(f"{what}: {err} -- retrying on {path}", RuntimeWarning, stacklevel=3)
        return True

    def __del__(self):
        h = getattr(self, "_h", None)
        if h is not None and h.value:
            for t in list(getattr(self, "_traces", ())):
                t.close()
            self._trace_cache = None
            self._h = None
            self._lib.tvr_model_destroy(h)

    def _stream(self) -> int:
        return torch.cuda.current_stream(self.device).cuda_stream

    def _check_range(self, what: str, force: bool = False) -> None:
        if self.gemm == "x2f16" and (force or self._range_depth == 0):
            _lib.check(self._lib.tvr_model_range_status(self._h, self._stream()), what)

    @contextlib.contextmanager
    def range_scope(self, what: str):
        self._range_depth += 1
        try:
            yield self
        except BaseException:
            self._range_depth -= 1
            raise
        self._range_depth -= 1
        self._check_range(what)

    def _op(self, name: str, *args):
        try:
            return getattr(self._ops, name)(*args)
        except ValueError:
            raise
        except RuntimeError as e:
            raise _lib.EngineError(str(e)) from e

    def trace(self, n_seqs: int, n_tokens: int) -> Trace:
        return Trace(self, max(n_seqs, 1), max(n_tokens, 1))

    def _sweep_trace(self, n_seqs: int, n_tokens: int) -> Trace:
        t = self._trace_cache
        if t is None or t.max_seqs < n_seqs or t.max_tokens < n_tokens:
            if t is not None:
                t.flush()
            self._trace_cache = None
            t = Trace(self, max(n_seqs, 1), max(n_tokens, 1), weak=True)
            self._trace_cache = t
        return t

    @staticmethod
    def _pack(seqs: Sequence[Sequence[int]]):
        lens = np.asarray([len(s) for s in seqs], dtype=np.int32)
        toks = np.asarray([int(x) for s in seqs for x in s], dtype=np.int32)
        return toks, lens

    def forward_clean(self, seqs: Sequence[Sequence[int]], targets: Optional[Sequence[int]] = None,
                      topk: int = 0, return_logits: bool = False, capture: bool = False,
                      trace: Optional[Trace] = None, defer: bool = False) -> Dict[str, torch.Tensor]:
        n = len(seqs)
        if n == 0:
            raise ValueError("no prompts")
        toks, lens = self._pack(seqs)
        tg = None
        if targets is not None:
            tg = np.asarray([-1 if t is None else int(t) for t in targets], dtype=np.int32)
            if tg.shape[0] != n:
                raise ValueError("targets must have one entry per prompt")
        if trace is not None and (trace.max_seqs < n or trace.max_tokens < int(lens.sum())):
            raise ValueError("trace too small for this batch")
        if defer and (trace is None or return_logits or capture):
            raise ValueError("defer needs a trace and no logits / capture")
# ... 321 lines not shown
```

Measured before the change: 19520 patched prompts/s.

## Keep row-pair-interleaved copies of exact-fp16 weights for the pingpong GEMM

When the model runs the exact-fp16 x2f16 path with interleaved activations, it allocates device copies of every layer's W1/W2 and the unembed weight in a row-pair-interleaved layout, then points the pingpong GEMM's weight-interleaved kernel variant at them. The layout matches the interleaved activation tiling, which is meant to make weight tile loads more contiguous in the ping-pong kernel. The cost is a second full copy of the fp16 weights in HBM plus a one-time conversion, with a fallback that skips the copy if allocation fails. An env var can force the old row layout.

```diff
diff --git a/include/tvr.h b/include/tvr.h
--- a/include/tvr.h
+++ b/include/tvr.h
@@ -88,6 +88,10 @@
 } tvr_exact16_layer;
 int tvr_model_set_exact16(tvr_model* model, const tvr_exact16_layer* layers );
 int tvr_model_set_exact16_unembed(tvr_model* model, const uint16_t* wu, const float* gf);
+#define TVR_W_IL_LAYERS 1
+#define TVR_W_IL_UNEMBED 2
+#define TVR_W_IL_NOMEM 4
+int32_t tvr_model_weight_layout(const tvr_model* model);
 
 int tvr_trace_create(tvr_model* model, int32_t max_seqs, int32_t max_tokens,
                      tvr_trace** out);
@@ -155,6 +159,7 @@
 #define TVR_ACT_X2F16_IL 0x12
 int tvr_act_rows(int32_t fmt, const float* a, int32_t lda, uint16_t* out, int32_t rows,
                  int32_t K, uint32_t* range_flag, void* stream);
+int tvr_weight_rows_il(const uint16_t* w, uint16_t* out, int32_t N, int32_t K, void* stream);
 int tvr_gemm_planar(int32_t fmt, const uint16_t* A, int32_t lda, const uint16_t* W,
                     int32_t ldw, size_t wps, float w_scale, const float* bias,
                     float* C, int32_t ldc, int32_t M, int32_t N, int32_t K,
diff --git a/task-vector-replication_amd/_lib.py b/task-vector-replication_amd/_lib.py
--- a/task-vector-replication_amd/_lib.py
+++ b/task-vector-replication_amd/_lib.py
@@ -90,6 +90,7 @@
 EPI_BIAS, EPI_GELU, EPI_RESID = 0, 1, 2
 FORM_PLAN, FORM_PLAIN, FORM_SPLITK, FORM_TAIL, FORM_STREAMK = 0, 1, 2, 3, 4
 SLICE_MODEL, SLICE_ON, SLICE_OFF = 0, 1, 2
+W_IL_LAYERS, W_IL_UNEMBED, W_IL_NOMEM = 1, 2, 4
 
 
 class CKernelStats(ctypes.Structure):
@@ -151,6 +152,9 @@
     "tvr_model_set_exact16": (ctypes.c_int, [ctypes.c_void_p, ctypes.c_void_p]),
     "tvr_model_set_exact16_unembed": (ctypes.c_int, [ctypes.c_void_p, ctypes.c_void_p, ctypes.c_void_p]),
     "tvr_model_get_gemm": (ctypes.c_int32, [ctypes.c_void_p]),
+    "tvr_model_weight_layout": (ctypes.c_int32, [ctypes.c_void_p]),
+    "tvr_weight_rows_il": (ctypes.c_int, [ctypes.c_void_p, ctypes.c_void_p, ctypes.c_int32, ctypes.c_int32,
+                                          ctypes.c_void_p]),
     "tvr_split_planes": (ctypes.c_int, [c_f32p, ctypes.c_void_p, ctypes.c_size_t, ctypes.c_void_p]),
     "tvr_gemm_x3bf16": (ctypes.c_int, [c_f32p, ctypes.c_int32, ctypes.c_void_p, ctypes.c_int32,
                                        ctypes.c_size_t, c_f32p, c_f32p, ctypes.c_int32, ctypes.c_int32,
diff --git a/task-vector-replication_amd/csrc/engine.hip b/task-vector-replication_amd/csrc/engine.hip
--- a/task-vector-replication_amd/csrc/engine.hip
+++ b/task-vector-replication_amd/csrc/engine.hip
@@ -80,8 +80,10 @@
   size_t wps = 0;
   float wscale = 1.0f;
   bool x16 = false;
+  const uint16_t* hil = nullptr;
   MatW rows(size_t elems) const {
-    return {f ? f + elems : nullptr, x ? x + elems : nullptr, h ? h + elems : nullptr, wps, wscale, x16};
+    return {f ? f + elems : nullptr, x ? x + elems : nullptr, h ? h + elems : nullptr, wps, wscale, x16,
+            hil ? hil + elems : nullptr};
   }
 };
 
@@ -139,6 +141,10 @@
   std::vector<const float*> g1, g2;
   MatW wux;
   const float* gf = nullptr;
+  uint16_t* w_il = nullptr;
+  uint16_t* wu_il = nullptr;
+  bool w_il_wanted = true;
+  bool w_il_nomem = false;
 };
 
 struct tvr_trace {
@@ -293,6 +299,10 @@
 bool act_layout_interleaved() {
   const char* e = getenv("TVR_ACT_LAYOUT");
   return !(e && std::string(e) == "planar");
+}
+bool w_layout_interleaved() {
+  const char* e = getenv("TVR_W_LAYOUT");
+  return !(e && std::string(e) == "rows");
 }
 int acts_fmt(const tvr_model* m) { return use_x16(m) && m->act_il ? (int)ACT_X2F16I : act_fmt(m); }
 
@@ -488,7 +498,8 @@
                                       std::to_string(g.epi) + ", fmt " + std::to_string(g.fmt) + ", vec " +
                                       std::to_string(g.vec) + ", stream-K " + std::to_string(g.skm) + ", sliced " +
                                       std::to_string(g.sl) + ", one weight plane " + std::to_string(g.wx) +
-                                      ", interleaved A " + std::to_string(g.ail));
+                                      ", interleaved A " + std::to_string(g.ail) + ", interleaved W " +
+                                      std::to_string(g.wil));
   };
   pl.skm = plan.sk_base >= 0;
   const bool whole_split = !pl.skm && plan.ksplit > 1, tail_split = !pl.skm && !whole_split && plan.tail_base > 0;
@@ -547,6 +558,9 @@
     return fail(TVR_ERR_UNSUPPORTED, "gemm: K, lda, ldw must be multiples of 32/4/4 (8 for planes, K of 64 for "
                                      "bf16; K=" + std::to_string(K) + ")");
   const bool wx = a_fmt == ACT_X2F16 && W.x16;
+  const bool wil = wx && ail && W.hil != nullptr && pp_wil_available();
+  MatW Wl = W;
+  if (wil) Wl.h = W.hil;
   bool vec = false, sl = false, skinny = false;
   PpLaunch pl;
   if (planar) {
@@ -563,7 +577,7 @@
         plan = force->plan;
       else if (m && vec && epi != EPI_STATS)
         plan = plan_pp_cached(m, M, N, K, a_fmt, epi, wx);
-      TVR_TRY(resolve_pp(PpForm{epi, a_fmt, vec || epi == EPI_STATS, false, sl, wx, ail}, plan, pl));
+      TVR_TRY(resolve_pp(PpForm{epi, a_fmt, vec || epi == EPI_STATS, false, sl, wx, ail, wil}, plan, pl));
     }
   }
   hipEvent_t ev0 = nullptr, ev1 = nullptr;
@@ -591,9 +605,9 @@
 #undef TVR_SK_F
 #undef TVR_SK
     } else {
-      if (pl.n == 0 || pl.base > 0) launch_pp(pl.whole, Ah, lda, W, ldw, M, N, K, ep, acc_scale, 0, pl.base, st);
+      if (pl.n == 0 || pl.base > 0) launch_pp(pl.whole, Ah, lda, Wl, ldw, M, N, K, ep, acc_scale, 0, pl.base, st);
       if (pl.n > 0)
-        TVR_TRY(launch_pp_partial(pl, Ah, lda, a_fmt, W, ldw, M, N, K, ep, acc_scale,
+        TVR_TRY(launch_pp_partial(pl, Ah, lda, a_fmt, Wl, ldw, M, N, K, ep, acc_scale,
                                   gemm_pingpong_grid(M, N) - pl.base, m, st));
     }
   } else {
@@ -645,6 +659,13 @@
     m->prof_recs.push_back({ev0, ev1, kind, 2.0 * M * N * (double)K,
                             abytes * M * (double)K + cbytes + wbytes * N * (double)K});
   }
+  return TVR_OK;
+}
+
+int w_from_row(const MatW& W, int r0, int ld, MatW& out) {
+  if (W.hil && (r0 & 1))
+    return fail(TVR_ERR_INTERNAL, "gemm: odd weight row offset " + std::to_string(r0) + " into a row-pair-interleaved plane");
+  out = W.rows((size_t)r0 * ld);
   return TVR_OK;
 }
 
@@ -1000,7 +1021,8 @@
   const int epi = fmt != ACT_F32 ? EPI_SPLIT_GELU_ACT : EPI_SPLIT_GELU;
   if (xn2) {
     if (!use_x16(m) || !act_is_x2(fmt)) return fail(TVR_ERR_INTERNAL, "launch_w1: gamma-scaled rows off the x16 path");
-    const MatW W = m->w1x[l].rows((size_t)c0 * d);
+    MatW W;
+    TVR_TRY(w_from_row(m->w1x[l], c0, d, W));
     const int qkv_end = 3 * d - c0;
     if (qkv_end <= 0)
       return launch_gemm(epi, xn2, d, fmt, W, d, M, N, d, ep, st, m);
@@ -1021,7 +1043,9 @@
     if (ep.out0m) e2.out0m = ep.out0m + qkv_end;
     e2.n_split = ep.n_split - qkv_end;
     if (e2.n_split < 0) return fail(TVR_ERR_INTERNAL, "launch_w1: MLP-in columns below the GELU split");
-    return launch_gemm(epi, xn2, d, fmt, W.rows((size_t)qkv_end * d), d, M, N - qkv_end, d, e2, st, m);
+    MatW W2;
+    TVR_TRY(w_from_row(W, qkv_end, d, W2));
+    return launch_gemm(epi, xn2, d, fmt, W2, d, M, N - qkv_end, d, e2, st, m);
   }
   const int nqk = fmt == ACT_BF16 && !m->w1qk.empty() ? std::min(std::max(2 * d - c0, 0), N) : 0;
   if (nqk > 0) {
@@ -1285,9 +1309,91 @@
   return TVR_OK;
 }
 
+static void free_w_il(tvr_model* m, bool layers, bool unembed) {
+  if (layers) {
+    if (m->w_il) (void)hipFree(m->w_il);
+    m->w_il = nullptr;
+    for (auto& w : m->w1x) w.hil = nullptr;
+    for (auto& w : m->w2x) w.hil = nullptr;
+  }
+  if (unembed) {
+    if (m->wu_il) (void)hipFree(m->wu_il);
+    m->wu_il = nullptr;
+    m->wux.hil = nullptr;
+  }
+  if (!m->w_il && !m->wu_il) m->w_il_nomem = false;
+}
+
+static int sync_w_il(tvr_model* m) {
+  const bool want = use_x16(m) && m->act_il && m->w_il_wanted && pp_wil_available();
+  if (!want) {
+    if (m->w_il || m->wu_il) TVR_HIP(hipDeviceSynchronize());
+    free_w_il(m, true, true);
+    return TVR_OK;
+  }
+  const tvr_config& c = m->cfg;
+  const int L = c.n_layers, d = c.d_model;
+  const dim3 grid(4096), block(256);
+  bool launched = false;
+  if (!m->w_il) {
+    const size_t n1 = w_il_halves(m->D1, d), n2 = w_il_halves(d, m->K2);
+    if (hipMalloc(&m->w_il, (size_t)L * (n1 + n2) * sizeof(uint16_t)) != hipSuccess) {
+      m->w_il = nullptr;
+      (void)hipGetLastError();
+      m->w_il_nomem = true;
+    } else {
+      uint16_t* p = m->w_il;
+      for (int l = 0; l < L; ++l) {
+        hipLaunchKernelGGL(weight_plane_il_kernel, grid, block, 0, 0, m->w1x[l].h, p, (size_t)m->D1, d);
+        m->w1x[l].hil = p;
+        p += n1;
+        hipLaunchKernelGGL(weight_plane_il_kernel, grid, block, 0, 0, m->w2x[l].h, p, (size_t)d, m->K2);
+        m->w2x[l].hil = p;
+        p += n2;
+      }
+      launched = true;
+    }
+  }
+  if (m->wux.h && !m->wu_il) {
+    if (hipMalloc(&m->wu_il, w_il_halves(c.d_vocab, d) * sizeof(uint16_t)) != hipSuccess) {
+      m->wu_il = nullptr;
+      (void)hipGetLastError();
+      m->w_il_nomem = true;
+    } else {
+      hipLaunchKernelGGL(weight_plane_il_kernel, grid, block, 0, 0, m->wux.h, m->wu_il, (size_t)c.d_vocab, d);
+      m->wux.hil = m->wu_il;
+      launched = true;
+    }
+  }
+  if (launched) {
+    hipError_t e = hipGetLastError();
+    if (e == hipSuccess) e = hipDeviceSynchronize();
+    if (e != hipSuccess) {
+      free_w_il(m, true, true);
+      return fail(TVR_ERR_HIP, std::string("interleaved weight copies: ") + hipGetErrorString(e));
+    }
+  }
+  return TVR_OK;
+}
+
+int32_t tvr_model_weight_layout(const tvr_model* m) {
+  if (!m) return -1;
+  return (m->w_il ? TVR_W_IL_LAYERS : 0) | (m->wu_il ? TVR_W_IL_UNEMBED : 0) | (m->w_il_nomem ? TVR_W_IL_NOMEM : 0);
+}
+
+int tvr_weight_rows_il(const uint16_t* w, uint16_t* out, int32_t N, int32_t K, void* stream) {
+  if (!w || !out || N <= 0 || K <= 0 || K % 32 != 0) return fail(TVR_ERR_INVALID, "tvr_weight_rows_il: bad argument");
+  const size_t n = w_il_halves(N, K);
+  hipLaunchKernelGGL(weight_plane_il_kernel, dim3((unsigned)std::min<size_t>((n + 255) / 256, 8192)), dim3(256), 0,
+                     (hipStream_t)stream, w, out, (size_t)N, K);
+  TVR_HIP(hipGetLastError());
+  return TVR_OK;
+}
+
 int tvr_model_destroy(tvr_model* m) {
   if (!m) return TVR_OK;
   (void)hipDeviceSynchronize();
+  free_w_il(m, true, true);
   if (m->rot_cos) (void)hipFree(m->rot_cos);
   if (m->rot_sin) (void)hipFree(m->rot_sin);
   if (m->d_w2s) (void)hipFree(m->d_w2s);
@@ -1324,14 +1430,18 @@
 int tvr_model_set_exact16_unembed(tvr_model* m, const uint16_t* wu, const float* gf) {
   if (!m) return fail(TVR_ERR_INVALID, "tvr_model_set_exact16_unembed: null model");
   if (!wu != !gf) return fail(TVR_ERR_INVALID, "tvr_model_set_exact16_unembed: give both arrays or neither");
+  if (m->wu_il) TVR_HIP(hipDeviceSynchronize());
+  free_w_il(m, false, true);
   m->wux = wu ? MatW{nullptr, nullptr, wu, 0, 1.0f, true} : MatW{};
   m->gf = gf;
-  return TVR_OK;
+  return sync_w_il(m);
 }
 
 int tvr_model_set_exact16(tvr_model* m, const tvr_exact16_layer* layers) {
   if (!m) return fail(TVR_ERR_INVALID, "tvr_model_set_exact16: null model");
   const tvr_config& c = m->cfg;
+  if (m->w_il || m->wu_il) TVR_HIP(hipDeviceSynchronize());
+  free_w_il(m, true, true);
   if (!layers) {
     const bool was = m->x16;
     m->x16 = false;
@@ -1357,6 +1467,7 @@
     m->g2.push_back(layers[l].g2);
   }
   m->x16 = true;
+  m->w_il_wanted = w_layout_interleaved();
   return replan_x2f16(m);
 }
 
@@ -1382,6 +1493,7 @@
   m->lin_mode = -1;
   m->lin_failed_mode = -1;
   m->gemm_mode = TVR_GEMM_F32;
+  TVR_TRY(sync_w_il(m));
   if (mode == TVR_GEMM_F32) return TVR_OK;
 
   const tvr_config& c = m->cfg;
@@ -1491,7 +1603,7 @@
   TVR_HIP(hipStreamSynchronize(st));
   m->gemm_mode = mode;
   m->act_il = act_layout_interleaved();
-  return TVR_OK;
+  return sync_w_il(m);
 }
 
 int tvr_model_range_status(tvr_model* m, void* stream) {
@@ -2235,8 +2347,9 @@
       rc = launch_gemm(EPI_BIAS, vg1, d, fmt, m->w1x[l], d, nv, q, d, ex, st, m);
       GemmEpi e2 = ex;
       e2.out0 = ex.out0 + q;
-      if (rc == TVR_OK)
-        rc = launch_gemm(EPI_BIAS, vg2, d, fmt, m->w1x[l].rows((size_t)q * d), d, nv, D1 - q, d, e2, st, m);
+      MatW Wq;
+      if (rc == TVR_OK) rc = w_from_row(m->w1x[l], q, d, Wq);
+      if (rc == TVR_OK) rc = launch_gemm(EPI_BIAS, vg2, d, fmt, Wq, d, nv, D1 - q, d, e2, st, m);
     }
   } else if (nqk > 0) {
     rc = launch_gemm(EPI_BIAS, cx.vact + d, d, ACT_F16, m->w1qk[l], d, nv, nqk, d, eg, st, m);
@@ -2600,7 +2713,12 @@
   if (!a) return bad("null args");
   if (a->fmt != TVR_GEMM_X2F16 && a->fmt != TVR_ACT_X2F16_IL && a->fmt != TVR_GEMM_BF16)
     return bad("unknown fmt " + std::to_string(a->fmt));
-  if (a->exact16 != 0 && a->exact16 != 1) return bad("exact16 must be 0 or 1");
+  if (a->exact16 < 0 || a->exact16 > 2) return bad("exact16 must be 0, 1 or 2");
+  if (a->exact16 == 2 && a->fmt != TVR_ACT_X2F16_IL)
+    return bad("exact16 must be 0 or 1 with this fmt: the row-pair-interleaved weight plane (2) takes the "
+               "interleaved activation layout");
+  if (a->exact16 == 2 && !pp_wil_available())
+    return fail(TVR_ERR_UNSUPPORTED, "tvr_gemm_launch: this build has no interleaved-weight kernel (TVR_PP_WX_WIDE 0)");
   if (a->epi != TVR_EPI_BIAS && a->epi != TVR_EPI_GELU && a->epi != TVR_EPI_RESID)
     return bad("unknown epi " + std::to_string(a->epi));
   if (a->form < TVR_FORM_PLAN || a->form > TVR_FORM_STREAMK) return bad("unknown form " + std::to_string(a->form));
@@ -2740,7 +2858,7 @@
   if (rc == TVR_OK) {
     const int epi = a->epi == TVR_EPI_BIAS ? EPI_BIAS : a->epi == TVR_EPI_GELU ? EPI_SPLIT_GELU_ACT : EPI_RESID;
     const int afmt = il ? ACT_X2F16I : x2 ? ACT_X2F16 : ACT_BF16;
-    MatW W{nullptr, nullptr, a->W, (size_t)a->wps, x2 ? a->w_scale : 1.0f, x16};
+    MatW W{nullptr, nullptr, a->W, (size_t)a->wps, x2 ? a->w_scale : 1.0f, x16, a->exact16 == 2 ? a->W : nullptr};
     rc = launch_gemm(epi, a->A, a->lda, afmt, W, a->ldw, M, N, K, e, st, il && !x16 ? nullptr : m, nullptr, &force);
     if (rc == TVR_OK) {
       const hipError_t err = hipGetLastError();
diff --git a/task-vector-replication_amd/csrc/gemm_pingpong.hpp b/task-vector-replication_amd/csrc/gemm_pingpong.hpp
--- a/task-vector-replication_amd/csrc/gemm_pingpong.hpp
+++ b/task-vector-replication_amd/csrc/gemm_pingpong.hpp
@@ -5,6 +5,7 @@
 #include <type_traits>
 
 #include "gemm_planar.hpp"
+#include "w_layout.hpp"
 
 namespace tvr {
 
@@ -724,9 +725,9 @@
         src[R][s] = Ab + plane * aps + (size_t)(ep.a_rows ? ep.a_rows[am] : am) * lda + chunk * 8;
         dst[R][s] = plane * PL + trow0 * (AIL ? ABK : BK);
       } else {
-        const int wn = min(n0 + row, N - 1);
+        const int wn = w_tile_row(n0, row, N);
         if constexpr (WIL)
-          src[R][s] = W + (size_t)(wn >> 1) * (2 * ldw) + (wn & 1) * 32 + chunk * 8;
+          src[R][s] = W + w_il_stage_offset(wn, chunk, ldw);
         else
           src[R][s] = W + (size_t)wn * ldw + chunk * 8;
         dst[R][s] = NPL * PL + trow0 * BK;
@@ -735,7 +736,7 @@
   }
   auto stage = [&](int R, int kt) {
     const bool live = kt < nk;
-    const int koff = live ? (kbeg + kt) * ((AIL && R < 2) || (WIL && R >= 2) ? 64 : BK) : 0;
+    const int koff = live ? (kbeg + kt) * (AIL && R < 2 ? 64 : WIL && R >= 2 ? W_IL_KTILE : BK) : 0;
     const int boff = (TWO ? kt % 3 : kt & 1) * BUF;
 #pragma unroll
     for (int s = 0; s < (R >= 2 ? WP : 2); ++s) glds16(src[R][s] + koff, lds + (live ? boff + dst[R][s] : DUMMY));
@@ -1098,11 +1099,14 @@
 struct PpForm {
   int epi, fmt;
   bool vec, skm, sl, wx, ail;
+  bool wil = false;
 };
 using PpKernel = void (*)(const uint16_t*, int, size_t, const uint16_t*, int, size_t, float, int, int, int, GemmEpi);
 
-constexpr bool pp_form_exists(int epi, int fmt, bool vec, bool skm, bool sl, bool wx, bool ail) {
+constexpr bool pp_wil_available() { return TVR_PP_WX_WIDE != 0; }
+constexpr bool pp_form_exists(int epi, int fmt, bool vec, bool skm, bool sl, bool wx, bool ail, bool wil = false) {
   if (fmt != ACT_X2F16 && (sl || wx || ail)) return false;
+  if (wil && !(wx && ail && pp_wil_available())) return false;
   if (ail && !wx && (epi != EPI_BIAS || skm)) return false;
   if (skm) return epi == EPI_BIAS && vec;
   switch (epi) {
@@ -1114,10 +1118,10 @@
   }
 }
 
-template <int EPI, int FMT, bool VEC, bool SKM, bool SL, bool WX, bool AIL>
+template <int EPI, int FMT, bool VEC, bool SKM, bool SL, bool WX, bool AIL, bool WIL>
 PpKernel pp_kernel_at() {
-  if constexpr (pp_form_exists(EPI, FMT, VEC, SKM, SL, WX, AIL))
-    return gemm_pingpong_kernel<EPI, FMT, VEC, 0, SKM, SL, WX, AIL>;
+  if constexpr (pp_form_exists(EPI, FMT, VEC, SKM, SL, WX, AIL, WIL))
+    return gemm_pingpong_kernel<EPI, FMT, VEC, 0, SKM, SL, WX, AIL, WIL>;
   else
     return nullptr;
 }
@@ -1128,9 +1132,9 @@
 template <int EPI>
 PpKernel pp_kernel_epi(const PpForm& f) {
   switch (f.fmt) {
-    case ACT_X2F16: return pp_kernel_at<EPI, ACT_X2F16>(f.vec, f.skm, f.sl, f.wx, f.ail);
-    case ACT_BF16: return pp_kernel_at<EPI, ACT_BF16>(f.vec, f.skm, f.sl, f.wx, f.ail);
-    case ACT_F16: return pp_kernel_at<EPI, ACT_F16>(f.vec, f.skm, f.sl, f.wx, f.ail);
+    case ACT_X2F16: return pp_kernel_at<EPI, ACT_X2F16>(f.vec, f.skm, f.sl, f.wx, f.ail, f.wil);
+    case ACT_BF16: return pp_kernel_at<EPI, ACT_BF16>(f.vec, f.skm, f.sl, f.wx, f.ail, f.wil);
+    case ACT_F16: return pp_kernel_at<EPI, ACT_F16>(f.vec, f.skm, f.sl, f.wx, f.ail, f.wil);
     default: return nullptr;
   }
 }
diff --git a/task-vector-replication_amd/csrc/w_layout.hpp b/task-vector-replication_amd/csrc/w_layout.hpp
--- /dev/null
+++ b/task-vector-replication_amd/csrc/w_layout.hpp
@@ -0,0 +1,38 @@
+#pragma once
+#include <stddef.h>
+#include <stdint.h>
+
+#if defined(__HIPCC__)
+#include <hip/hip_runtime.h>
+#define TVR_HD __host__ __device__ __forceinline__
+#else
+#define TVR_HD inline
+#endif
+
+namespace tvr {
+
+constexpr int W_IL_KTILE = 64;
+
+TVR_HD size_t w_il_halves(size_t N, size_t ldw) { return (N + 1) / 2 * 2 * ldw; }
+
+TVR_HD size_t w_il_offset(size_t n, size_t k, size_t ldw) {
+  return (n >> 1) * 2 * ldw + (k >> 5) * W_IL_KTILE + (n & 1) * 32 + (k & 31);
+}
+
+TVR_HD int w_tile_row(int n0, int row, int N) { return n0 + row < N - 1 ? n0 + row : N - 1; }
+
+TVR_HD size_t w_il_stage_offset(int wn, int chunk, int ldw) {
+  return (size_t)(wn >> 1) * (2 * ldw) + (wn & 1) * 32 + chunk * 8;
+}
+
+#if defined(__HIPCC__)
+__global__ void weight_plane_il_kernel(const uint16_t* __restrict__ w, uint16_t* __restrict__ out, size_t N, int K) {
+  const size_t n = (N + 1) / 2 * 2 * K;
+  for (size_t i = blockIdx.x * (size_t)blockDim.x + threadIdx.x; i < n; i += (size_t)gridDim.x * blockDim.x) {
+    const size_t r = i / K, c = i % K;
+    out[w_il_offset(r, c, K)] = r < N ? w[i] : (uint16_t)0;
+  }
+}
+#endif
+
+}
diff --git a/task-vector-replication_amd/model.py b/task-vector-replication_amd/model.py
--- a/task-vector-replication_amd/model.py
+++ b/task-vector-replication_amd/model.py
@@ -253,6 +253,10 @@
                 self.exact16 = bool(on)
                 self.gemm = _lib.GEMM_NAMES.get(self._lib.tvr_model_get_gemm(self._h), self.gemm)
 
+    @property
+    def weight_layout(self) -> int:
+        return int(self._lib.tvr_model_weight_layout(self._h))
+
     def _fall_back(self, what: str, err: Exception) -> bool:
         if self.gemm != "x2f16":
             return False
```

Result: faster. 19900 patched prompts/s, median of 6 (+1.9%).
